# ns1labs/pktvisor

Hardware: AMD Instinct MI355X
Metric: Mpkt/s device-resident (Net+DNS handler parse) (higher is better)
Workload: dtype u8; 1 GPU; C2: Net+DNS handlers, 64 B UDP (Eth+IPv4+UDP+22 B), Zipf IPs, host_spec 10.x.x.x/8; records_per_gpu=10000000, handlers=net v1 + dns v1 (default groups), parallelism=dp1

## Files before the change

### include/pvgpu.h

```cpp
#ifndef PVGPU_H
#define PVGPU_H

#include <stddef.h>
#include <stdint.h>

#ifdef __cplusplus
extern "C" {
#endif

typedef struct pv_ctx pv_ctx;

enum pv_status {
    PV_OK = 0,
    PV_EINVAL = -1,
    PV_EHIP = -2,
    PV_ECAPACITY = -3,
    PV_EUNSUPPORTED = -4,
    PV_ENODEV = -5
};

enum pv_net_group { PV_NET_COUNTERS = 1u << 0, PV_NET_CARDINALITY = 1u << 1, PV_NET_TOP_GEO = 1u << 2, PV_NET_TOP_IPS = 1u << 3 };
enum pv_dns_group {
    PV_DNS_CARDINALITY = 1u << 0, PV_DNS_COUNTERS = 1u << 1, PV_DNS_QUANTILES = 1u << 2, PV_DNS_HISTOGRAMS = 1u << 3,
    PV_DNS_TRANSACTIONS = 1u << 4, PV_DNS_TOP_ECS = 1u << 5, PV_DNS_TOP_QNAMES = 1u << 6,
// ... 151 lines not shown
int pv_merge_hints(pv_ctx *ctx, uint64_t *open_queries, uint64_t *xact_values);
int pv_slow_values_export(pv_ctx *ctx, uint8_t **buf, size_t *bytes);
int pv_slow_finish(pv_ctx *ctx, const uint8_t *const *bufs, const size_t *sizes, uint32_t nranks);
int pv_values_export(pv_ctx *ctx, uint8_t **buf, size_t *bytes);
int pv_values_merge(pv_ctx *ctx, const uint8_t *buf, size_t bytes);
int pv_window_periods(pv_ctx *ctx, int part, uint32_t *slots, int64_t *start_sec, uint32_t max_n, uint32_t *n);
int pv_advance_windows(pv_ctx *ctx, int part, const int64_t *thresh, uint32_t n);
int pv_dns_event_seconds(pv_ctx *ctx, const uint8_t *d_recs, const uint32_t *d_offs, const pv_index_info *info,
                         const uint32_t *sc_idx, const uint32_t *sc_sec, int64_t *secs, uint32_t max, uint32_t *n);
int pv_plan_dns_draws(pv_ctx *ctx, uint64_t *draws);
int pv_sample_skip(pv_ctx *ctx, uint64_t net_draws, uint64_t dns_draws);
int pv_dns_event_seconds_host(pv_ctx *ctx, const uint8_t *recs, size_t bytes, int64_t *secs, uint32_t max, uint32_t *n);
int pv_shard_cuts(const uint8_t *recs, size_t bytes, const uint32_t *offs, uint64_t n, uint32_t linktype, uint32_t ts_nano,
                  uint32_t world, uint64_t *cuts);


int pv_set_start_tstamp(pv_ctx *ctx, int64_t sec, int64_t nsec);
int pv_set_end_tstamp(pv_ctx *ctx, int64_t sec, int64_t nsec);
int pv_synchronize(pv_ctx *ctx);
int pv_reset(pv_ctx *ctx);

int pv_window_json(pv_ctx *ctx, uint32_t period, int merged, char **out);
void pv_free(void *p);

#define PV_HANDLER_NET 1u
#define PV_HANDLER_DNS 2u
#define PV_PERIOD_AUTO 0xFFFFFFFFu
int pv_window_prometheus(pv_ctx *ctx, uint32_t period, uint32_t handlers, const char *const *label_keys,
                         const char *const *label_values, uint32_t n_labels, char **out);
int pv_window_opentelemetry(pv_ctx *ctx, uint32_t period, uint32_t handlers, const char *const *label_keys,
                            const char *const *label_values, uint32_t n_labels, uint8_t **out, size_t *bytes);
int pv_add_static_label(const char *key, const char *value);

int pv_check_period_shift(pv_ctx *ctx, int64_t sec, int64_t nsec);

typedef struct pv_bucket pv_bucket;
int pv_bucket_merge(pv_ctx *ctx, uint32_t handler, pv_bucket **bucket, uint32_t period, int prometheus, int merged);
int pv_bucket_json(pv_ctx *ctx, const pv_bucket *bucket, char **out);
int pv_bucket_prometheus(pv_ctx *ctx, const pv_bucket *bucket, const char *const *label_keys,
                         const char *const *label_values, uint32_t n_labels, char **out);
int pv_bucket_opentelemetry(pv_ctx *ctx, const pv_bucket *bucket, const char *const *label_keys,
                            const char *const *label_values, uint32_t n_labels, uint8_t **out, size_t *bytes);
void pv_bucket_free(pv_bucket *bucket);

int pv_state_regions(pv_ctx *ctx, void **sum_ptr, size_t *sum_bytes, void **min_ptr, size_t *min_bytes);
int pv_set_global_base(pv_ctx *ctx, uint64_t base);
enum pv_reduce_op { PV_REDUCE_SUM = 0, PV_REDUCE_MIN = 1 };
typedef struct pv_region {
    void *ptr;
    uint64_t words;
    uint32_t op;
    uint32_t pad;
} pv_region;
int pv_window_regions(pv_ctx *ctx, pv_region *regions, uint32_t max, uint32_t *n);

#define PV_COMM_ID_BYTES 128
int pv_comm_unique_id(uint8_t id[PV_COMM_ID_BYTES]);
int pv_comm_init(pv_ctx *ctx, const uint8_t id[PV_COMM_ID_BYTES], int nranks, int rank);
int pv_comm_allreduce_window(pv_ctx *ctx);
int pv_comm_allgather(pv_ctx *ctx, const void *buf, size_t bytes, uint8_t **out, uint64_t *sizes);
int pv_comm_destroy(pv_ctx *ctx);
int pv_export_topn(pv_ctx *ctx, uint8_t **buf, size_t *bytes);
int pv_merge_topn(pv_ctx *ctx, const uint8_t *buf, size_t bytes);

int pv_comm_merge_topn(pv_ctx *ctx);
int pv_topn_x_export(pv_ctx *ctx, uint32_t ranks, uint32_t rank, uint8_t **blob, size_t *bytes);
int pv_topn_x_import(pv_ctx *ctx, uint32_t ranks, uint32_t rank, const uint8_t *const *blobs, const size_t *sizes);
int pv_topn_x_candidates(pv_ctx *ctx, uint8_t **blob, size_t *bytes);
int pv_topn_x_names(pv_ctx *ctx, const uint8_t *const *cands, const size_t *sizes, uint32_t n, uint8_t **blob, size_t *bytes);
int pv_topn_x_view(pv_ctx *ctx, const uint8_t *const *cands, const size_t *csizes, const uint8_t *const *names,
                   const size_t *nsizes, uint32_t n);

typedef int (*pv_allreduce_fn)(uint64_t *buf, size_t n, int op, void *user);
int pv_values_x_select(pv_ctx *ctx, pv_allreduce_fn allreduce, void *user);
int pv_comm_values_select(pv_ctx *ctx);
int pv_slow_x_finish(pv_ctx *ctx, pv_allreduce_fn allreduce, void *user);
int pv_comm_slow_finish(pv_ctx *ctx);

int pv_set_kernel_timing(pv_ctx *ctx, uint32_t every);
const char *pv_net_kernel_name(pv_ctx *ctx);
int pv_kernel_timing(pv_ctx *ctx, double *total_ms, uint64_t *launches, int reset);
int pv_chain_stats(pv_ctx *ctx, uint64_t out[4], int reset);
int pv_fuse_stats(pv_ctx *ctx, uint64_t out[2], int reset);

typedef struct pv_geodb pv_geodb;
enum pv_geodb_kind { PV_GEODB_CITY = 0, PV_GEODB_ASN = 1 };
int pv_geodb_open(const uint8_t *bytes, size_t len, uint32_t kind, pv_geodb **db);
int pv_geodb_open_file(const char *path, uint32_t kind, pv_geodb **db);
void pv_geodb_close(pv_geodb *db);
const char *pv_geodb_last_error(void);
uint32_t pv_geodb_entries(const pv_geodb *db);
uint64_t pv_geodb_hash(const pv_geodb *db);
int pv_geodb_entry(const pv_geodb *db, uint32_t id, const char **name, const char **lat, const char **lon);
int pv_geodb_lookup(const pv_geodb *db, const uint8_t *addrs, size_t n, uint32_t addr_len, uint32_t *ids);
int pv_set_geodb(pv_ctx *ctx, const pv_geodb *city, const pv_geodb *asn);
typedef struct pv_net_filters {
    uint32_t geoloc_notfound;
    uint32_t asn_notfound;
    uint32_t only_geoloc_prefix_set;
    uint32_t n_geoloc_prefixes;
    const char *const *geoloc_prefixes;
    uint32_t only_asn_number_set;
    uint32_t n_asn_numbers;
    const char *const *asn_numbers;
} pv_net_filters;
int pv_set_net_filters(pv_ctx *ctx, const pv_net_filters *f);

#define PV_HANDLER_DHCP 4u
typedef struct pv_dhcp_config {
    uint32_t xact_ttl_ms;
    uint32_t recorded_stream;
    uint32_t max_events;
} pv_dhcp_config;
int pv_set_dhcp(pv_ctx *ctx, const pv_dhcp_config *cfg);
int pv_dhcp_timing(pv_ctx *ctx, double *scan_ms, uint64_t *launches, int reset);

#define PV_HANDLER_BGP 8u
typedef struct pv_bgp_config {
    uint32_t recorded_stream;
    uint32_t max_events;
} pv_bgp_config;
int pv_set_bgp(pv_ctx *ctx, const pv_bgp_config *cfg);
int pv_bgp_timing(pv_ctx *ctx, double *scan_ms, uint64_t *launches, int reset);
int pv_geodb_hashes(pv_ctx *ctx, uint64_t hashes[2]);
int pv_geodb_lookup_device(pv_ctx *ctx, uint32_t kind, const uint8_t *addrs, size_t n, uint32_t addr_len, uint32_t *ids);

#ifdef __cplusplus
}
#endif
#endif
```

### pktvisor_amd/__init__.py

```python
from __future__ import annotations

import ctypes
import json
import os
import struct
from typing import Optional

import numpy as np

HERE = os.path.dirname(os.path.abspath(__file__))
LIB_PATH = os.path.join(HERE, "libpvgpu.so")

PV_NET_COUNTERS, PV_NET_CARDINALITY, PV_NET_TOP_GEO, PV_NET_TOP_IPS = 1, 2, 4, 8
DNS_GROUPS = {"cardinality": 1 << 0, "counters": 1 << 1, "quantiles": 1 << 2, "histograms": 1 << 3,
              "dns_transaction": 1 << 4, "top_ecs": 1 << 5, "top_qnames": 1 << 6, "top_qnames_details": 1 << 7,
              "top_ports": 1 << 8}
NET_GROUPS = {"counters": 1, "cardinality": 2, "top_geo": 4, "top_ips": 8}
DNS_DEFAULT = sum(DNS_GROUPS[g] for g in ("cardinality", "counters", "quantiles", "dns_transaction", "top_qnames",
                                          "top_ports"))
NET_DEFAULT = 15


from pktvisor_amd.config import PvError

# ... 61 lines not shown
        if k in cfg and not isinstance(cfg[k], bool):
            raise ConfigError(f"wrong type for key: {k}")
    for k in ("only_qtype", "only_qname", "only_qname_suffix"):
        if k in cfg and (not isinstance(cfg[k], (list, tuple)) or not all(isinstance(x, str) for x in cfg[k])):
            raise ConfigError(f"wrong type for key: {k}")
    if cfg.get("exclude_noerror"):
        out["exclude_noerror"] = 1
    elif "only_rcode" in cfg:
        v = cfg["only_rcode"]
        if isinstance(v, bool) or not isinstance(v, (int, list, tuple)):
            raise ConfigError("DnsStreamHandler: wrong value type for only_rcode filter. It should be an integer or an array")
        if isinstance(v, int):
            if _dns_code(0, str(v)) is None:
                raise ConfigError("DnsStreamHandler: only_rcode filter contained an invalid/unsupported rcode")
            codes = [v]
        else:
            codes = []
            for r in v:
                c = _dns_code(0, r)
                if c is None:
                    raise ConfigError(f"DnsStreamHandler: only_rcode filter contained an invalid/unsupported rcode: {r}")
                codes.append(c)
        for c in codes:
            if c > 15:
                raise ConfigError("DnsStreamHandler: only_rcode filter contained an invalid/unsupported rcode")
            out["only_rcode_mask"] |= 1 << c
    if cfg.get("only_queries"):
        out["only_queries"] = 1
    if cfg.get("only_responses"):
        out["only_responses"] = 1
    if cfg.get("only_dnssec_response"):
        out["only_dnssec_response"] = 1
    if cfg.get("public_suffix_list"):
        out["public_suffix_list"] = 1
    if "answer_count" in cfg:
        v = cfg["answer_count"]
        if isinstance(v, bool) or not isinstance(v, int):
            raise ConfigError("DnsStreamHandler: wrong value type for answer_count filter. It should be an integer")
        out["answer_count"] = v
    for q in cfg.get("only_qtype", []):
        c = _dns_code(1, q)
        if c is None:
            raise ConfigError(f"DnsStreamHandler: only_qtype filter contained an invalid/unsupported qtype: {q}")
        out["only_qtype"].append(c)
    out["only_qname"] = [str(q).lower() for q in cfg.get("only_qname", [])]
    if out["only_qname"] and out["only_rcode_mask"] and not v2:
        raise ConfigError("DnsStreamHandler: only_qname and only_rcode both install an input predicate: use one")
    if len(out["only_qname"]) > 8 or any(not q or len(q) > 255 for q in out["only_qname"]):
        raise ConfigError("DnsStreamHandler: only_qname: 1..8 names of 1..255 characters")
    out["only_qname_suffix"] = [str(q).lower() for q in cfg.get("only_qname_suffix", [])]
    if len(out["only_qname_suffix"]) > 4:
        raise ConfigError("DnsStreamHandler: only_qname_suffix: at most 4 suffixes")
    if len(out["only_qtype"]) > 16:
        raise ConfigError("DnsStreamHandler: only_qtype: at most 16 qtypes")
    return out


class pv_index_info(ctypes.Structure):
    _fields_ = [("n_records", ctypes.c_uint64), ("bytes_used", ctypes.c_uint64), ("first_sec", ctypes.c_int64),
                ("first_nsec", ctypes.c_int64), ("last_sec", ctypes.c_int64), ("last_nsec", ctypes.c_int64),
                ("monotone", ctypes.c_uint32), ("n_sec_changes", ctypes.c_uint32)]


EXPORTS = ["pv_version", "pv_device_count", "pv_create", "pv_destroy", "pv_last_error", "pv_index_records",
           "pv_index_records_device",
           "pv_process_device", "pv_process_host", "pv_set_start_tstamp", "pv_set_end_tstamp", "pv_synchronize",
           "pv_reset", "pv_window_json", "pv_free", "pv_state_regions", "pv_set_global_base", "pv_export_topn",
           "pv_merge_topn", "pv_kernel_timing", "pv_set_kernel_timing", "pv_window_regions", "pv_index_records_mt", "pv_host_register",
           "pv_host_unregister", "pv_ingest_timing", "pv_edge_export", "pv_edge_merge", "pv_values_export",
           "pv_values_merge", "pv_window_periods", "pv_set_dns_filters", "pv_dns_code", "pv_advance_windows",
           "pv_dns_event_seconds", "pv_dns_event_seconds_host", "pv_comm_unique_id", "pv_comm_init",
           "pv_comm_allreduce_window", "pv_comm_allgather", "pv_comm_destroy", "pv_process_dnstap", "pv_dnstap_count",
           "pv_pcapng_records", "pv_tpacket3_block_records", "pv_window_prometheus", "pv_add_static_label",
           "pv_window_opentelemetry", "pv_check_period_shift", "pv_bucket_merge", "pv_bucket_json",
           "pv_bucket_prometheus", "pv_bucket_opentelemetry", "pv_bucket_free", "pv_set_slow_defer",
           "pv_slow_values_export", "pv_slow_finish", "pv_edge_carry", "pv_merge_hints", "pv_set_end_of_capture", "pv_shard_cuts", "pv_net_kernel_name",
           "pv_plan_dns_draws", "pv_sample_skip", "pv_set_tcp_reassembly_limit", "pv_set_tcp_exact_lru", "pv_set_dnstap_only_hosts",
           "pv_afpacket_open", "pv_afpacket_attach", "pv_afpacket_run", "pv_afpacket_start", "pv_afpacket_stop",
           "pv_afpacket_stats", "pv_afpacket_close", "pv_afpacket_last_error", "pv_set_bpf", "pv_bpf_validate",
           "pv_bpf_run", "pv_bpf_filter_records", "pv_comm_merge_topn", "pv_topn_x_export", "pv_topn_x_import",
           "pv_topn_x_candidates", "pv_topn_x_names", "pv_topn_x_view", "pv_values_x_select", "pv_comm_values_select",
           "pv_slow_x_finish", "pv_comm_slow_finish", "pv_geodb_open", "pv_geodb_open_file", "pv_geodb_close",
           "pv_geodb_last_error", "pv_geodb_entries", "pv_geodb_hash", "pv_geodb_hashes", "pv_set_net_filters", "pv_geodb_entry", "pv_geodb_lookup", "pv_set_geodb",
           "pv_geodb_lookup_device", "pv_set_dhcp", "pv_dhcp_timing", "pv_set_bgp", "pv_bgp_timing", "pv_chain_stats", "pv_fuse_stats"]
PV_GEODB_CITY, PV_GEODB_ASN = 0, 1
ALLREDUCE_FN = ctypes.CFUNCTYPE(ctypes.c_int, ctypes.POINTER(ctypes.c_uint64), ctypes.c_size_t, ctypes.c_int, ctypes.c_void_p)
PV_HANDLER_NET, PV_HANDLER_DNS, PV_HANDLER_DHCP, PV_HANDLER_BGP = 1, 2, 4, 8
_HANDLER_BITS = {"net": PV_HANDLER_NET, "dns": PV_HANDLER_DNS, "dhcp": PV_HANDLER_DHCP, "bgp": PV_HANDLER_BGP}
PV_PERIOD_AUTO = 0xFFFFFFFF
PART_NET, PART_DNS = 0, 1
PV_REDUCE_SUM, PV_REDUCE_MIN = 0, 1


class pv_bpf_insn(ctypes.Structure):
    _fields_ = [("code", ctypes.c_uint16), ("jt", ctypes.c_uint8), ("jf", ctypes.c_uint8), ("k", ctypes.c_uint32)]


def bpf_program(insns):
    arr = (pv_bpf_insn * max(1, len(insns)))()
    for i, (c, jt, jf, k) in enumerate(insns):
        arr[i] = pv_bpf_insn(c, jt, jf, k & 0xFFFFFFFF)
    return arr


def bpf_filter(recs: bytes, insns) -> bytes:
    lib = load_library()
    prog = bpf_program(insns)
    src = np.frombuffer(recs, dtype=np.uint8)
    out = np.empty(max(1, len(recs)), dtype=np.uint8)
    nb = ctypes.c_size_t()
    rc = lib.pv_bpf_filter_records(prog, len(insns), src.ctypes.data if len(recs) else None, len(recs), out.ctypes.data,
                                   ctypes.byref(nb), None)
    if rc:
        raise PvError(f"pv_bpf_filter_records failed ({rc}): invalid BPF program")
    return out[:nb.value].tobytes()


class pv_afpacket_config(ctypes.Structure):
    _fields_ = [("interface", ctypes.c_char_p), ("fanout_group_id", ctypes.c_int), ("block_size", ctypes.c_uint32),
                ("frame_size", ctypes.c_uint32), ("num_blocks", ctypes.c_uint32), ("bpf_insns", ctypes.c_void_p),
                ("bpf_len", ctypes.c_uint32), ("batch_bytes", ctypes.c_uint32), ("flush_ms", ctypes.c_uint32)]


class pv_afpacket_counters(ctypes.Structure):
    _fields_ = [(k, ctypes.c_uint64) for k in ("blocks", "packets", "batches", "bytes", "kernel_packets", "kernel_drops",
                                              "kernel_freezes")]


AFPACKET_SINK = ctypes.CFUNCTYPE(ctypes.c_int, ctypes.c_void_p, ctypes.c_void_p, ctypes.c_size_t, ctypes.c_uint64)


class pv_region(ctypes.Structure):
    _fields_ = [("ptr", ctypes.c_void_p), ("words", ctypes.c_uint64), ("op", ctypes.c_uint32), ("pad", ctypes.c_uint32)]

_lib = None


def load_library(path: str = LIB_PATH) -> ctypes.CDLL:
    global _lib
    if _lib is not None:
        return _lib
    path = os.environ.get("PVGPU_LIB", path)
    if not os.path.exists(path):
        raise PvError(f"{path} missing: run `make -C pktvisor_amd` (or __graft_entry__.build())")
    lib = ctypes.CDLL(path)
    P, U32, U64, I64 = ctypes.c_void_p, ctypes.c_uint32, ctypes.c_uint64, ctypes.c_int64
    lib.pv_version.restype = ctypes.c_char_p
    lib.pv_device_count.argtypes = [ctypes.POINTER(ctypes.c_int)]
    lib.pv_create.argtypes = [ctypes.POINTER(pv_config), ctypes.POINTER(P)]
    lib.pv_destroy.argtypes = [P]
    lib.pv_destroy.restype = None
    lib.pv_last_error.argtypes = [P]
    lib.pv_last_error.restype = ctypes.c_char_p
    lib.pv_index_records.argtypes = [P, ctypes.c_size_t, U32, P, U64, P, P, U32, ctypes.POINTER(pv_index_info)]
    lib.pv_index_records_device.argtypes = [P, P, ctypes.c_size_t, P, U64, P, P, U32, ctypes.POINTER(pv_index_info)]
    lib.pv_process_device.argtypes = [P, P, P, ctypes.POINTER(pv_index_info), P, P, P]
    lib.pv_index_records_mt.argtypes = [P, ctypes.c_size_t, U32, P, U64, P, P, U32, ctypes.POINTER(pv_index_info),
                                        U32]
    lib.pv_process_host.argtypes = [P, P, ctypes.c_size_t]
    lib.pv_host_register.argtypes = [P, ctypes.c_size_t]
    lib.pv_host_unregister.argtypes = [P]
    lib.pv_ingest_timing.argtypes = [P, ctypes.POINTER(ctypes.c_double), ctypes.c_int]
    lib.pv_set_start_tstamp.argtypes = [P, I64, I64]
    lib.pv_set_end_tstamp.argtypes = [P, I64, I64]
    lib.pv_synchronize.argtypes = [P]
    lib.pv_reset.argtypes = [P]
    lib.pv_window_json.argtypes = [P, U32, ctypes.c_int, ctypes.POINTER(P)]
# ... 24 lines not shown
    lib.pv_dns_event_seconds_host.argtypes = [P, P, ctypes.c_size_t, P, U32, ctypes.POINTER(U32)]
    lib.pv_kernel_timing.argtypes = [P, ctypes.POINTER(ctypes.c_double), ctypes.POINTER(U64), ctypes.c_int]
    lib.pv_set_kernel_timing.argtypes = [P, ctypes.c_uint32]
    lib.pv_edge_export.argtypes = [P, ctypes.POINTER(P), ctypes.POINTER(ctypes.c_size_t)]
    lib.pv_edge_merge.argtypes = [P, P, P, U32, U32]
    lib.pv_set_slow_defer.argtypes = [P, ctypes.c_int]
    lib.pv_plan_dns_draws.argtypes = [P, ctypes.POINTER(ctypes.c_uint64)]
    lib.pv_sample_skip.argtypes = [P, ctypes.c_uint64, ctypes.c_uint64]
    lib.pv_net_kernel_name.argtypes = [P]
    lib.pv_net_kernel_name.restype = ctypes.c_char_p
    lib.pv_shard_cuts.argtypes = [P, ctypes.c_size_t, P, ctypes.c_uint64, U32, U32, U32, P]
    lib.pv_edge_carry.argtypes = [P, P, ctypes.c_size_t, ctypes.POINTER(P), ctypes.POINTER(ctypes.c_size_t)]
    lib.pv_merge_hints.argtypes = [P, ctypes.POINTER(ctypes.c_uint64), ctypes.POINTER(ctypes.c_uint64)]
    lib.pv_set_end_of_capture.argtypes = [P, ctypes.c_int]
    lib.pv_slow_values_export.argtypes = [P, ctypes.POINTER(P), ctypes.POINTER(ctypes.c_size_t)]
    lib.pv_slow_finish.argtypes = [P, P, P, U32]
    lib.pv_values_export.argtypes = [P, ctypes.POINTER(P), ctypes.POINTER(ctypes.c_size_t)]
    lib.pv_values_merge.argtypes = [P, P, ctypes.c_size_t]
    lib.pv_window_periods.argtypes = [P, ctypes.c_int, P, P, U32, ctypes.POINTER(U32)]
    lib.pv_set_dns_filters.argtypes = [P, ctypes.POINTER(pv_dns_filters)]
    lib.pv_set_tcp_reassembly_limit.argtypes = [P, ctypes.c_uint64]
    lib.pv_set_tcp_exact_lru.argtypes = [P, ctypes.c_int]
    lib.pv_set_bpf.argtypes = [P, P, U32]
    lib.pv_bpf_validate.argtypes = [P, U32]
    lib.pv_bpf_run.argtypes = [P, P, U32, U32]
    lib.pv_bpf_run.restype = ctypes.c_uint32
    lib.pv_bpf_filter_records.argtypes = [P, U32, P, ctypes.c_size_t, P, ctypes.POINTER(ctypes.c_size_t), P]
    lib.pv_set_dnstap_only_hosts.argtypes = [P, ctypes.c_char_p]
    lib.pv_dns_code.argtypes = [ctypes.c_int, ctypes.c_char_p, ctypes.POINTER(U32)]
    lib.pv_comm_unique_id.argtypes = [P]
    lib.pv_comm_init.argtypes = [P, P, ctypes.c_int, ctypes.c_int]
    lib.pv_comm_allreduce_window.argtypes = [P]
    lib.pv_comm_allgather.argtypes = [P, P, ctypes.c_size_t, ctypes.POINTER(P), P]
    lib.pv_comm_destroy.argtypes = [P]
    lib.pv_comm_merge_topn.argtypes = [P]
    lib.pv_topn_x_export.argtypes = [P, U32, U32, ctypes.POINTER(P), ctypes.POINTER(ctypes.c_size_t)]
    lib.pv_topn_x_import.argtypes = [P, U32, U32, P, P]
    lib.pv_topn_x_candidates.argtypes = [P, ctypes.POINTER(P), ctypes.POINTER(ctypes.c_size_t)]
    lib.pv_topn_x_names.argtypes = [P, P, P, U32, ctypes.POINTER(P), ctypes.POINTER(ctypes.c_size_t)]
    lib.pv_topn_x_view.argtypes = [P, P, P, P, P, U32]
    lib.pv_values_x_select.argtypes = [P, ALLREDUCE_FN, P]
    lib.pv_comm_values_select.argtypes = [P]
    lib.pv_slow_x_finish.argtypes = [P, ALLREDUCE_FN, P]
    lib.pv_comm_slow_finish.argtypes = [P]
    lib.pv_process_dnstap.argtypes = [P, P, ctypes.c_size_t, U32]
    lib.pv_tpacket3_block_records.argtypes = [P, ctypes.c_size_t, P, ctypes.c_size_t, ctypes.POINTER(ctypes.c_size_t),
                                              ctypes.POINTER(U64)]
    lib.pv_pcapng_records.argtypes = [P, ctypes.c_size_t, P, ctypes.c_size_t, ctypes.POINTER(ctypes.c_size_t),
                                      ctypes.POINTER(U32), ctypes.POINTER(U64)]
    lib.pv_dnstap_count.argtypes = [P, ctypes.c_size_t, ctypes.POINTER(U32), ctypes.POINTER(U32)]
    lib.pv_afpacket_open.argtypes = [ctypes.POINTER(pv_afpacket_config), ctypes.POINTER(P)]
    lib.pv_afpacket_attach.argtypes = [P, U32, U32, ctypes.c_int, ctypes.POINTER(pv_afpacket_config), ctypes.POINTER(P)]
    lib.pv_afpacket_run.argtypes = [P, AFPACKET_SINK, P]
    lib.pv_afpacket_start.argtypes = [P, P]
    lib.pv_afpacket_stop.argtypes = [P]
    lib.pv_afpacket_stats.argtypes = [P, ctypes.POINTER(pv_afpacket_counters)]
    lib.pv_afpacket_close.argtypes = [P]
    lib.pv_afpacket_close.restype = None
    lib.pv_afpacket_last_error.restype = ctypes.c_char_p
    lib.pv_geodb_open.argtypes = [P, ctypes.c_size_t, U32, ctypes.POINTER(P)]
    lib.pv_geodb_open_file.argtypes = [ctypes.c_char_p, U32, ctypes.POINTER(P)]
    lib.pv_geodb_close.argtypes = [P]
    lib.pv_geodb_close.restype = None
    lib.pv_geodb_last_error.restype = ctypes.c_char_p
    lib.pv_geodb_entries.argtypes = [P]
    lib.pv_geodb_entries.restype = U32
    lib.pv_set_net_filters.argtypes = [P, ctypes.POINTER(pv_net_filters)]
    lib.pv_geodb_hashes.argtypes = [P, ctypes.POINTER(ctypes.c_uint64)]
    lib.pv_geodb_hash.argtypes = [P]
    lib.pv_geodb_hash.restype = U64
    lib.pv_geodb_entry.argtypes = [P, U32, ctypes.POINTER(ctypes.c_char_p), ctypes.POINTER(ctypes.c_char_p),
                                   ctypes.POINTER(ctypes.c_char_p)]
    lib.pv_geodb_lookup.argtypes = [P, P, ctypes.c_size_t, U32, P]
    lib.pv_set_geodb.argtypes = [P, P, P]
    lib.pv_geodb_lookup_device.argtypes = [P, U32, P, ctypes.c_size_t, U32, P]
    lib.pv_set_dhcp.argtypes = [P, ctypes.POINTER(pv_dhcp_config)]
    lib.pv_dhcp_timing.argtypes = [P, ctypes.POINTER(ctypes.c_double), ctypes.POINTER(U64), ctypes.c_int]
    lib.pv_set_bgp.argtypes = [P, ctypes.POINTER(pv_bgp_config)]
    lib.pv_bgp_timing.argtypes = [P, ctypes.POINTER(ctypes.c_double), ctypes.POINTER(U64), ctypes.c_int]
    if hasattr(lib, "pv_chain_stats"):
        lib.pv_chain_stats.argtypes = [P, ctypes.POINTER(U64), ctypes.c_int]
    if hasattr(lib, "pv_fuse_stats"):
        lib.pv_fuse_stats.argtypes = [P, ctypes.POINTER(U64), ctypes.c_int]
    _lib = lib
    return lib


def comm_unique_id() -> bytes:
    buf = ctypes.create_string_buffer(128)
    if load_library().pv_comm_unique_id(buf) != 0:
        raise PvError("pv_comm_unique_id failed")
    return buf.raw


def device_count() -> int:
    n = ctypes.c_int(0)
    load_library().pv_device_count(ctypes.byref(n))
    return n.value


def pcapng_records(data: bytes):
    lib = load_library()
    buf = np.frombuffer(data, dtype=np.uint8)
    nb, lt, nr = ctypes.c_size_t(0), ctypes.c_uint32(0), ctypes.c_uint64(0)
    rc = lib.pv_pcapng_records(buf.ctypes.data, buf.nbytes, None, 0, ctypes.byref(nb), ctypes.byref(lt), ctypes.byref(nr))
    if rc:
        raise PvError("Cannot open pcap/pcapng file" + (" (interfaces with different linktypes)" if rc == -7 else ""))
    out = np.empty(nb.value, dtype=np.uint8)
    rc = lib.pv_pcapng_records(buf.ctypes.data, buf.nbytes, out.ctypes.data, out.nbytes, ctypes.byref(nb),
                               ctypes.byref(lt), ctypes.byref(nr))
    if rc:
        raise PvError(f"pv_pcapng_records failed ({rc})")
    return lt.value, out.tobytes()


def read_pcap(path: str):
    with open(path, "rb") as f:
        data = f.read()
    if len(data) >= 12 and struct.unpack_from("<I", data, 0)[0] == 0x0A0D0D0A:
        lt, recs = pcapng_records(data)
        return lt, 1, recs
    if len(data) < 24:
        raise PvError("Cannot open pcap/pcapng file")
    magic = struct.unpack_from("<I", data, 0)[0]
    if magic not in (0xA1B2C3D4, 0xA1B23C4D):
        raise PvError("Cannot open pcap/pcapng file (only little-endian classic pcap is supported)")
    linktype = struct.unpack_from("<I", data, 20)[0]
    return linktype, int(magic == 0xA1B23C4D), data[24:]


def tpacket3_records(blocks, out_cap: int = 1 << 26) -> bytes:
    lib = load_library()
    out = np.empty(out_cap, dtype=np.uint8)
    used, n = ctypes.c_size_t(0), ctypes.c_uint64(0)
    for b in blocks:
        buf = np.frombuffer(b, dtype=np.uint8)
        rc = lib.pv_tpacket3_block_records(buf.ctypes.data, buf.nbytes, out.ctypes.data, out.nbytes, ctypes.byref(used),
                                           ctypes.byref(n))
        if rc:
            raise PvError(f"pv_tpacket3_block_records failed ({rc})")
    return out[: used.value].tobytes()


def dnstap_count(frames: bytes):
    nf, ne = ctypes.c_uint32(0), ctypes.c_uint32(0)
    buf = np.frombuffer(frames, dtype=np.uint8)
    load_library().pv_dnstap_count(buf.ctypes.data, buf.nbytes, ctypes.byref(nf), ctypes.byref(ne))
    return nf.value, ne.value


def dnstap_reader(path: str, periods: int = 1, only_hosts: Optional[list] = None, **kw) -> dict:
    with open(path, "rb") as f:
        frames = f.read()
    h = PvHandlers(num_periods=periods, **kw)
    try:
        if only_hosts is not None:
            h._check(h.lib.pv_set_dnstap_only_hosts(h.ctx, ",".join(only_hosts).encode()), "pv_set_dnstap_only_hosts")
        h.process_dnstap(frames)
        key = f"{1 if periods == 1 else periods}m"
        return {key: h.window_json(0 if periods == 1 else periods, merged=periods != 1)}
    finally:
        h.close()


def pcap_file_bytes(records: bytes, linktype: int = 1, ts_nano: int = 0) -> bytes:
    magic = 0xA1B23C4D if ts_nano else 0xA1B2C3D4
# ... 254 lines not shown
        self._host = host_spec.encode() if host_spec else None
        cfg = pv_config(self._host, num_periods, topn_count, xact_ttl_ms, net_groups, dns_groups, linktype, ts_nano,
                        device, table_log2, max_records, topn_percentile_threshold, net_filter_all, net2_groups,
                        dns2_groups, deep_sample_rate)
        self.num_periods = num_periods
        self.device = device
        self.ctx = ctypes.c_void_p()
        rc = self.lib.pv_create(ctypes.byref(cfg), ctypes.byref(self.ctx))
        if rc:
            msg = self.lib.pv_last_error(self.ctx).decode() if self.ctx else "pv_create"
            self.lib.pv_destroy(self.ctx)
            self.ctx = None
            raise PvError(f"pv_create failed ({rc}): {msg}")
        if filt:
            f = pv_dns_filters(filt["exclude_noerror"], filt["only_rcode_mask"], filt["answer_count"],
                               filt["only_queries"], filt["only_responses"], len(filt["only_qtype"]))
            for k, q in enumerate(filt["only_qtype"]):
                f.qtypes[k] = q
            f.only_dnssec_response = filt["only_dnssec_response"]
            f.filter_all = filt.get("filter_all", 0)
            f.public_suffix_list = filt.get("public_suffix_list", 0)
            f.v2 = filt.get("v2", 0)
            f.xact_dirs_disabled = filt.get("xact_dirs_disabled", 0)
            if filt["only_qname"]:
                self._qnames = (ctypes.c_char_p * len(filt["only_qname"]))(*[q.encode() for q in filt["only_qname"]])
                f.n_qnames = len(filt["only_qname"])
                f.qnames = ctypes.cast(self._qnames, ctypes.POINTER(ctypes.c_char_p))
            if filt["only_qname_suffix"]:
                sx = filt["only_qname_suffix"]
                self._qsfx = (ctypes.c_char_p * len(sx))(*[q.encode() for q in sx])
                f.n_qname_suffixes = len(sx)
                f.qname_suffixes = ctypes.cast(self._qsfx, ctypes.POINTER(ctypes.c_char_p))
            self._check(self.lib.pv_set_dns_filters(self.ctx, ctypes.byref(f)), "pv_set_dns_filters")
        self.tcp_exact = bool(tcp_exact_lru or tcp_packet_reassembly_cache_limit)
        if tcp_packet_reassembly_cache_limit:
            self._check(self.lib.pv_set_tcp_reassembly_limit(self.ctx, int(tcp_packet_reassembly_cache_limit)),
                        "pv_set_tcp_reassembly_limit")
        if tcp_exact_lru:
            self._check(self.lib.pv_set_tcp_exact_lru(self.ctx, 1), "pv_set_tcp_exact_lru")
        if bpf:
            self.set_bpf(bpf)
        if geo_city_db is not None or geo_asn_db is not None:
            self.set_geodb(geo_city_db, geo_asn_db)
        if net_filters:
            self.set_net_filters(**net_filters)
        self.dhcp_attached = False
        if dhcp is not None:
            self.set_dhcp(dhcp["xact_ttl_ms"], dhcp["recorded_stream"], dhcp_max_events)

        self.bgp_attached = False
        if bgp is not None:
            self.set_bgp(bgp["recorded_stream"], bgp_max_events)

    def set_bgp(self, recorded_stream: bool = False, max_events: int = 0):
        cfg = pv_bgp_config(int(bool(recorded_stream)), int(max_events))
        self._check(self.lib.pv_set_bgp(self.ctx, ctypes.byref(cfg)), "pv_set_bgp")
        self.bgp_attached = True

    def bgp_timing(self, reset: bool = False):
        ms, n = ctypes.c_double(), ctypes.c_uint64()
        self._check(self.lib.pv_bgp_timing(self.ctx, ctypes.byref(ms), ctypes.byref(n), int(reset)), "pv_bgp_timing")
        return ms.value, n.value

    def set_dhcp(self, xact_ttl_ms: int = 0, recorded_stream: bool = False, max_events: int = 0):
        cfg = pv_dhcp_config(int(xact_ttl_ms), int(bool(recorded_stream)), int(max_events))
        self._check(self.lib.pv_set_dhcp(self.ctx, ctypes.byref(cfg)), "pv_set_dhcp")
        self.dhcp_attached = True

    def dhcp_timing(self, reset: bool = False):
        ms, n = ctypes.c_double(), ctypes.c_uint64()
        self._check(self.lib.pv_dhcp_timing(self.ctx, ctypes.byref(ms), ctypes.byref(n), int(reset)), "pv_dhcp_timing")
        return ms.value, n.value

    def chain_stats(self, reset: bool = False):
        out = (ctypes.c_uint64 * 4)()
        self._check(self.lib.pv_chain_stats(self.ctx, out, int(reset)), "pv_chain_stats")
        return tuple(int(v) for v in out)

    def fuse_stats(self, reset: bool = False):
        out = (ctypes.c_uint64 * 2)()
        self._check(self.lib.pv_fuse_stats(self.ctx, out, int(reset)), "pv_fuse_stats")
        return tuple(int(v) for v in out)

    def set_net_filters(self, geoloc_notfound=False, asn_notfound=False, only_geoloc_prefix=None, only_asn_number=None):
        f = pv_net_filters(int(bool(geoloc_notfound)), int(bool(asn_notfound)))
        keep = []
        for name, lst in (("geoloc_prefixes", only_geoloc_prefix), ("asn_numbers", only_asn_number)):
            if lst is None:
                continue
            arr = (ctypes.c_char_p * max(1, len(lst)))(*[str(x).encode() for x in lst])
            keep.append(arr)
            setattr(f, name, ctypes.cast(arr, ctypes.POINTER(ctypes.c_char_p)))
            setattr(f, "n_" + name, len(lst))
            setattr(f, "only_geoloc_prefix_set" if name == "geoloc_prefixes" else "only_asn_number_set", 1)
        self._check(self.lib.pv_set_net_filters(self.ctx, ctypes.byref(f)), "pv_set_net_filters")

    def set_geodb(self, city=None, asn=None):
        own = []
        dbs = []
        for src, kind in ((city, "city"), (asn, "asn")):
            if src is not None and not isinstance(src, GeoDB):
                src = GeoDB(src, kind)
                own.append(src)
            dbs.append(src)
        try:
            self._check(self.lib.pv_set_geodb(self.ctx, dbs[0].ptr if dbs[0] else None, dbs[1].ptr if dbs[1] else None),
                        "pv_set_geodb")
            hs = (ctypes.c_uint64 * 2)()
            self._check(self.lib.pv_geodb_hashes(self.ctx, hs), "pv_geodb_hashes")
            self.geo_hashes = [int(hs[0]), int(hs[1])]
        finally:
            for d in own:
                d.close()

    def geo_lookup_device(self, kind: str, addrs, addr_len: int) -> np.ndarray:
        buf = _packed_addrs(addrs, addr_len)
        ids = np.empty(buf.size // addr_len, dtype=np.uint32)
        self._check(self.lib.pv_geodb_lookup_device(self.ctx, PV_GEODB_CITY if kind == "city" else PV_GEODB_ASN,
                                                    buf.ctypes.data, ids.size, addr_len, ids.ctypes.data),
                    "pv_geodb_lookup_device")
        return ids

    def set_bpf(self, insns):
        self._bpf = bpf_program(insns or [])
        self._check(self.lib.pv_set_bpf(self.ctx, self._bpf, len(insns or [])), "pv_set_bpf")

    def _check(self, rc, what):
        if rc:
            raise PvError(f"{what} failed ({rc}): {self.lib.pv_last_error(self.ctx).decode()}")

    def close(self):
        if self.ctx:
            self.lib.pv_destroy(self.ctx)
            self.ctx = None

    def __del__(self):
        try:
            self.close()
        except Exception:
            pass

    def process_host(self, recs):
        buf = recs if isinstance(recs, np.ndarray) else np.frombuffer(recs, dtype=np.uint8)
        self._check(self.lib.pv_process_host(self.ctx, buf.ctypes.data, buf.nbytes), "pv_process_host")

    def set_end_of_capture(self, on: bool = True):
        self._check(self.lib.pv_set_end_of_capture(self.ctx, int(on)), "pv_set_end_of_capture")

    def process_dnstap(self, frames):
        buf = frames if isinstance(frames, np.ndarray) else np.frombuffer(frames, dtype=np.uint8)
        self._check(self.lib.pv_process_dnstap(self.ctx, buf.ctypes.data, buf.nbytes, self.dnstap_mask),
                    "pv_process_dnstap")

    def index_device(self, recs, max_records: Optional[int] = None, max_changes: int = 1 << 16):
        buf = np.frombuffer(recs, dtype=np.uint8) if not isinstance(recs, np.ndarray) else recs
        if max_records is None:
            max_records = max(1, len(buf) // 16)
        offs = np.empty(max_records, dtype=np.uint32)
        sci = np.empty(max_changes, dtype=np.uint32)
        scs = np.empty(max_changes, dtype=np.uint32)
        info = pv_index_info()
        self._check(self.lib.pv_index_records_device(self.ctx, buf.ctypes.data, len(buf), offs.ctypes.data, max_records,
                                                     sci.ctypes.data, scs.ctypes.data, max_changes, ctypes.byref(info)),
                    "pv_index_records_device")
        return offs[: info.n_records], sci, scs, info

# ... 348 lines not shown
```

### pktvisor_amd/csrc/pv_host.cpp

```cpp
#include "pv_host.h"

namespace {

int parse_host_spec(pv_ctx *c, const char *spec)
{
    if (!spec) return 0;
    std::string s = spec;
    size_t pos = 0;
    while (pos < s.size()) {
        size_t e = s.find(',', pos);
        std::string host = s.substr(pos, e == std::string::npos ? std::string::npos : e - pos);
        pos = e == std::string::npos ? s.size() : e + 1;
        if (host.empty()) continue;
        size_t d = host.find('/');
        if (d == std::string::npos) return c->fail(PV_EINVAL, "invalid CIDR: %s", host.c_str());
        std::string ip = host.substr(0, d), cs = host.substr(d + 1);
        if (cs.empty() || !std::all_of(cs.begin(), cs.end(), ::isdigit)) return c->fail(PV_EINVAL, "invalid CIDR: %s", host.c_str());
        int cidr = atoi(cs.c_str());
        if (ip.find(':') != std::string::npos) {
            if (cidr < 0 || cidr > 128) return c->fail(PV_EINVAL, "invalid CIDR: %s", host.c_str());
            if (c->nets.n6 >= PV_MAX_SUBNETS) return c->fail(PV_EINVAL, "too many host subnets");
            uint8_t a[16];
            if (inet_pton(AF_INET6, ip.c_str(), a) != 1) return c->fail(PV_EINVAL, "invalid IPv6 address: %s", ip.c_str());
            memcpy(c->nets.v6_addr[c->nets.n6], a, 16);
// ... 2044 lines not shown
    P.iplog32 = c->d_iplog32;
    P.ipdir = c->d_ipdir;
    P.ipx_cnt = c->d_ipx_cnt;
    P.ipx_rep = c->d_ipx_rep;
    P.trash = c->d_trash;
    if ((uint64_t)grid * 4 > PV_TRASH_WAVES) return c->fail(PV_ECAPACITY, "grid of %u workgroups exceeds the trash area", grid);
    P.cb = c->d_cb;
    P.cb_cnt = c->d_cb_cnt;
    P.cb_hm = c->d_cb_cnt + 32768;
    P.stamps = c->d_stamps;
    P.dq = c->d_dq;
    P.dq_cnt = c->d_dq_cnt;
    static const char *force = getenv("PV_NET_KERNEL");
    const bool general = P.n_shift || P.net_filter_all || P.gfilt || P.dbg || P.ndeep_net || c->tcp_exact_on() ||
                         (force && !strcmp(force, "general"));
    const uint32_t reg_grid = std::min<uint32_t>(grid, (uint32_t)(c->cus * c->reg_wg_per_cu));
    const uint64_t per_wave = ((uint64_t)P.wt_per_block / 4 + 1) * ((grid + reg_grid - 1) / reg_grid);
    const bool lean = !general && P.linktype == 1 && P.nets.n4 <= 2 && P.skip_before == 0 && per_wave < 65535 &&
                      !(force && !strcmp(force, "ns"));
    P.ip_compact = lean ? 1u : 0u;
    P.ip_base = ((uint64_t)P.slot_of[0] << 60) | ((uint64_t)TM_IPV4 << 56) |
                ((uint64_t)((c->net_groups & PV_NET_CARDINALITY) ? 1 : 0) << 33);
    const bool tc = (c->dev_net_groups() & PV_NET_TOP_IPS) != 0;
    {
        const char *fan = getenv("PV_CB_FAN"), *cmp = getenv("PV_CB_COMPACT");
        P.cb_compact = cmp && atoi(cmp) == 0 ? 0u : 1u;
        uint32_t pick = c->cb_fan;
        if (P.cb_compact && lean && tc && !c->net2_groups && c->cb_plain) {
            const uint32_t f = std::min<uint32_t>(3u, 65535u / (P.wt_per_block * 64u));
            if (f > 1 && (grid + f - 1) / f >= (uint32_t)c->cus) pick = f;
        }
        P.cb_fan = fan ? std::max(1u, std::min(8u, (uint32_t)atoi(fan))) : pick;
        while (P.cb_fan > 1 && (uint64_t)P.cb_fan * P.mq_cap >= (1u << 24)) P.cb_fan--;
        P.cb_grid = (grid + P.cb_fan - 1) / P.cb_fan;
    }
    const bool span = lean && tc && force && !strcmp(force, "span");
    bool plain = lean && !(force && !strcmp(force, "span")) && c->cb_plain && !c->net2_groups && !c->geo_counting();
    if (plain) {
        const char *pc = getenv("PV_PLAIN_CHAIN");
        if (pc && atoi(pc) == 0) plain = false;
    }
    P.plain_chain = plain ? 1u : 0u;
    bool fuse = plain && tc && P.cb_fan > 1 && P.cb_grid == reg_grid && c->reg_log2 <= 10;
    if (fuse) {
        const char *fp = getenv("PV_FUSE_PLAIN");
        if (fp && atoi(fp) == 0) fuse = false;
    }
    {
        const char *nc = getenv("PV_NET_CONTIG");
        P.net_contig = nc && atoi(nc) != 0 && lean && P.cb_fan > 1 && P.cb_grid == reg_grid ? 1u : 0u;
    }
    if (lean) {
        if (c->slow_cap < P.n) {
            if (c->d_slow) hipFree(c->d_slow);
            c->d_slow = nullptr;
            c->slow_cap = 0;
            if (!hip_ok(e = hipMalloc(&c->d_slow, (size_t)(P.n + PV_MAX_GRID) * 4))) return c->hipfail(e, "deferred record list");
            c->slow_cap = P.n;
        }
        P.slow_list = c->d_slow;
        P.slow_cnt = c->d_slow + c->slow_cap;
    }
    if (c->dns_groups & PV_DNS_TOP_ECS) {
        if (c->ecs_cap < P.n) {
            if (c->d_ecs) hipFree(c->d_ecs);
            c->d_ecs = nullptr;
            c->ecs_cap = 0;
            if (!hip_ok(e = hipMalloc(&c->d_ecs, (size_t)P.n * sizeof(uint4)))) return c->hipfail(e, "top_ecs list");
            c->ecs_cap = P.n;
        }
        P.ecs_list = reinterpret_cast<uint32_t *>(c->d_ecs);
        P.ecs_cap = (uint32_t)c->ecs_cap;
    }
    *c->h_params = P;
    if (!hip_ok(e = fill_and_upload(c, c->d_params, c->h_params, sizeof P, st)))
        return c->hipfail(e, "parameter upload");
    c->net_kernel = general ? "pv_net_kernel"
                            : (lean ? (span ? "pv_net_kernel_span" : (tc ? "pv_net_kernel_reg_tc" : "pv_net_kernel_reg"))
                                    : "pv_net_kernel_ns");
    const PvParams *dp = (const PvParams *)c->d_params;
    const bool timed = n && c->timing_every && (c->timing_ctr++ % c->timing_every) == 0;
    hipEvent_t e0 = timed ? c->ev_start : nullptr, e1 = timed ? c->ev_stop : nullptr;
    if (timed) fuse = false;
    if (P.gfilt && n) {
        PvGeoArgs G{};
        for (int k = 0; k < 2; k++) {
            const pv_ctx::GeoAttach &g = c->geo[k];
            if (!g.on) continue;
            G.tree[k] = g.d_tree;
            G.node_count[k] = g.node_count;
            G.start4[k] = g.start4;
            G.ip_version[k] = g.ip_version;
            G.entries[k] = (uint32_t)g.dict.size();
        }
        hipLaunchKernelGGL(pv_geo_verdict, dim3((uint32_t)((P.n + 255) / 256)), dim3(256), 0, st, dp, G,
                           (const uint8_t *)(c->nf_on[0] ? c->d_nf_pass[0] : nullptr),
                           (const uint8_t *)(c->nf_on[1] ? c->d_nf_pass[1] : nullptr), c->d_gfilt);
    }
    if (!n) {  }
    else if (general) hipExtLaunchKernelGGL(pv_net_kernel, dim3(grid), dim3(PV_NET_THREADS), 0, st, e0, e1, 0, dp);
    else if (lean) {
        hipEvent_t l1 = plain ? e1 : (hipEvent_t) nullptr;
        if (fuse) hipLaunchKernelGGL(pv_net_combine_plain, dim3(P.cb_grid), dim3(PV_CB_THREADS), 0, st, dp);
        else if (span) hipExtLaunchKernelGGL(pv_net_kernel_span, dim3(reg_grid), dim3(PV_NET_THREADS), 0, st, e0, l1, 0, dp);
        else if (tc) hipExtLaunchKernelGGL(pv_net_kernel_reg_tc, dim3(reg_grid), dim3(PV_NET_THREADS), 0, st, e0, l1, 0, dp);
        else hipExtLaunchKernelGGL(pv_net_kernel_reg, dim3(reg_grid), dim3(PV_NET_THREADS), 0, st, e0, l1, 0, dp);
        if (!plain) hipExtLaunchKernelGGL(pv_net_slow_list, dim3(c->cus * 2), dim3(256), 0, st, (hipEvent_t) nullptr, e1, 0, dp);
    }
    else hipExtLaunchKernelGGL(pv_net_kernel_ns, dim3(grid), dim3(PV_NET_THREADS), 0, st, e0, e1, 0, dp);
    e = hipGetLastError();
    if (e != hipSuccess) return c->hipfail(e, "launch pv_net_kernel");
    static int cb_threads = 0;
    if (!cb_threads) {
        hipFuncAttributes fa{};
        cb_threads = hipFuncGetAttributes(&fa, reinterpret_cast<const void *>(pv_topn_combine)) == hipSuccess ? fa.maxThreadsPerBlock
                                                                                                             : PV_CB_THREADS;
    }
    const bool sfx = (P.f_flags & (PVDF_ONLY_QSUFFIX | PVDF_PSL)) != 0;
    auto dns_stage = [&]() {
        if (sfx) hipLaunchKernelGGL(pv_dns_suffix, dim3(grid), dim3(256), 0, st, (const PvParams *)c->d_params);
        const uint32_t dns_grid = std::min<uint32_t>(grid, (uint32_t)(c->cus * c->dns_wg_per_cu));
        if (sfx)
            hipLaunchKernelGGL(pv_dns_kernel_sfx, dim3(dns_grid), dim3(64 * PV_DNS_WAVES), 0, st, (const PvParams *)c->d_params);
        else if (P.f_flags)
            hipLaunchKernelGGL(pv_dns_kernel_f, dim3(dns_grid), dim3(64 * PV_DNS_WAVES), 0, st, (const PvParams *)c->d_params);
        else
            hipLaunchKernelGGL(pv_dns_kernel, dim3(dns_grid), dim3(64 * PV_DNS_WAVES), 0, st, (const PvParams *)c->d_params);
        if (c->dns_groups & PV_DNS_TOP_ECS)
            hipLaunchKernelGGL(pv_dns_ecs, dim3((uint32_t)c->cus * 2), dim3(256), 0, st, (const PvParams *)c->d_params);
        if (c->net2_groups) hipLaunchKernelGGL(pv_net2_kernel, dim3(grid), dim3(256), 0, st, (const PvParams *)c->d_params);
    };
    auto topn_stage = [&](bool combined = false) {
        if (!combined)
            hipLaunchKernelGGL(c->reg_log2 <= 10 ? pv_topn_combine : pv_topn_combine_r12, dim3(P.cb_grid), dim3(cb_threads), 0, st,
                               (const PvParams *)c->d_params);
        if (c->geo_counting()) {
            PvGeoArgs G{};
            for (int k = 0; k < 2; k++) {
                const pv_ctx::GeoAttach &g = c->geo[k];
                if (!g.on) continue;
                G.tree[k] = g.d_tree;
                G.cnt[k] = g.d_cnt;
                G.node_count[k] = g.node_count;
                G.start4[k] = g.start4;
                G.ip_version[k] = g.ip_version;
                G.entries[k] = (uint32_t)g.dict.size();
            }
            hipLaunchKernelGGL(pv_geo_count, dim3(std::min<uint32_t>(P.cb_grid, (uint32_t)c->cus * 8)), dim3(256), 0, st,
                               (const PvParams *)c->d_params, G);
        }
        hipLaunchKernelGGL(pv_topn_merge, dim3(2u << c->reg_log2), dim3(pv_topn_merge_threads()), 0, st, (const PvParams *)c->d_params);
    };
    auto names_stage = [&]() {
        hipLaunchKernelGGL(sfx ? pv_topn_names_sfx : pv_topn_names, dim3((uint32_t)c->cus * 2), dim3(256), 0, st,
                           (const PvParams *)c->d_params);
    };
    uint32_t status[ST_WORDS];
    auto read_status = [&]() -> hipError_t {
        hipError_t r = hipGetLastError();
        if (r != hipSuccess) return r;
        if ((r = hipMemcpyAsync(c->h_status, c->d_status, ST_RB_WORDS * 4, hipMemcpyDeviceToHost, st)) != hipSuccess) return r;
        if ((r = hipStreamSynchronize(st)) != hipSuccess) return r;
        memcpy(status, c->h_status, sizeof status);
        return hipSuccess;
    };
    if (!n) {
    } else if (!plain) {
        dns_stage();
        topn_stage();
        names_stage();
        c->chain_n[3]++;
    } else {
        topn_stage(fuse);
        c->chain_n[0]++;
        if (fuse) c->fuse_n[0]++;
    }

    HP(14);
    if (!hip_ok(e = read_status())) return c->hipfail(e, "kernel execution");
    if (plain && (status[ST_NDNS] || status[ST_NSLOW])) {
        c->chain_n[1]++;
        if (fuse) c->fuse_n[1]++;
        P.plain_chain = 0;
        c->h_params->plain_chain = 0;
        if (!hip_ok(e = upload_params(c->d_params, c->h_params, sizeof P, st))) return c->hipfail(e, "parameter upload");
        hipLaunchKernelGGL(pv_net_slow_list, dim3(c->cus * 2), dim3(256), 0, st, dp);
        dns_stage();
        topn_stage();
        names_stage();
        if (!hip_ok(e = read_status())) return c->hipfail(e, "kernel execution");
    } else if (plain && status[ST_NNEW]) {
        c->chain_n[2]++;
        names_stage();
        if (!hip_ok(e = read_status())) return c->hipfail(e, "kernel execution");
    }
    if (n) {
        c->dns_heavy = (uint64_t)status[ST_NDNS] * 2 > n;
        c->cb_plain = lean && status[ST_NDNS] == 0 && status[ST_NSLOW] == 0;
    }
    if (status[ST_FLAGS] & PVF_NAMES_PENDING) {
        for (uint32_t t = 0; t < PV_TABLES; t++)
            hipLaunchKernelGGL(pv_topn_name_fix, dim3((uint32_t)c->cus * 4), dim3(256), 0, st, (const PvParams *)c->d_params, t);
        if (!hip_ok(e = hipGetLastError()) || !hip_ok(e = hipStreamSynchronize(st))) return c->hipfail(e, "pending names");
        if (getenv("PV_NAMEFIX_TRACE")) fprintf(stderr, "pv: pending top-N names written (pv_topn_name_fix)\n");
    }
    HP(4);
    {
        float ms = 0;
        if (timed && hipEventElapsedTime(&ms, c->ev_start, c->ev_stop) == hipSuccess) { c->kernel_ms += ms; c->kernel_launches++; }
    }
    if (!c->tcp_pre) {
        if (int rc = tcp_stage(c, d_recs, d_offs, n, status[ST_TSEG], status[ST_TSEG_BYTES], first_sec, false, st)) return rc;
    }
    const uint32_t gt = tcp_pass(c, P, a, a + nord, st, c->h_params + 1);
    if (gt) {
        if (P.want_events)
            hipLaunchKernelGGL(pv_xact_compact, dim3(gt), dim3(256), 0, st, (const PvParams *)c->d_params, grid,
                               status[ST_NKEYS]);
        if (!hip_ok(e = hipGetLastError())) return c->hipfail(e, "launch pv_dns_tcp");
        if (!hip_ok(e = hipMemcpyAsync(c->h_status, c->d_status, ST_RB_WORDS * 4, hipMemcpyDeviceToHost, st)) ||
            !hip_ok(e = hipStreamSynchronize(st)))
            return c->hipfail(e, "TCP DNS pass");
        memcpy(status, c->h_status, sizeof status);
    }
    for (uint32_t k = 0; k <= P.n_shift; k++) c->net.clean[P.slot_of[k]] = false;
    if (status[ST_NDNS] || gt)
        for (uint32_t k = 0; k <= P.n_dshift; k++) c->dns.clean[P.dslot_of[k]] = false;
    bool drained = false;
    if (int rc = drain_overflow(c, st, true, &drained)) return rc;
    uint32_t flags = status[ST_FLAGS];
    if (drained && !hip_ok(e = hipMemcpy(&flags, c->d_status + ST_FLAGS, 4, hipMemcpyDeviceToHost))) return c->hipfail(e, "status");
    if (flags & PVF_TABLE_FULL) return c->fail(PV_ECAPACITY, "top-N table full: raise table_log2");
    if (flags & PVF_ARENA_FULL) return c->fail(PV_ECAPACITY, "top-N name arena full");
    if (getenv("PV_TSTAMPS")) {
        std::vector<uint64_t> tv(65536 + (2u << c->reg_log2) * 8);
        if (hip_ok(hipMemcpy(tv.data(), c->d_stamps + (1u << 20), tv.size() * 8, hipMemcpyDeviceToHost))) {
            double cs[8] = {0}, ms[8] = {0};
            uint64_t nm = 0;
            const uint32_t cg = P.cb_grid;
            for (uint32_t w = 0; w < cg; w++)
                for (int k = 0; k < 8; k++) cs[k] += (double)tv[w * 8 + k];
            for (uint32_t w = 0; w < (2u << c->reg_log2); w++) {
                const uint64_t *m = &tv[65536 + w * 8];
                if (!m[0] && !m[1]) continue;
                nm++;
                for (int k = 0; k < 8; k++) ms[k] += (double)m[k];
            }
            fprintf(stderr, "pv_tstamps combine (%u wg): init=%.0f insert=%.0f count=%.0f scan=%.0f out=%.0f | merge (%lu wg): "
                            "runs=%.0f load=%.0f insert=%.0f names=%.0f wb=%.0f\n",
                    cg, cs[0] / cg, cs[1] / cg, cs[2] / cg, cs[3] / cg, cs[4] / cg, (unsigned long)nm,
                    ms[0] / std::max<uint64_t>(nm, 1), ms[1] / std::max<uint64_t>(nm, 1), ms[2] / std::max<uint64_t>(nm, 1),
                    ms[3] / std::max<uint64_t>(nm, 1), ms[4] / std::max<uint64_t>(nm, 1));
            hipMemset(c->d_stamps + (1u << 20), 0, tv.size() * 8);
        }
        std::vector<uint64_t> nv((size_t)reg_grid * 4);
        int khz = 0;
        hipDeviceGetAttribute(&khz, hipDeviceAttributeWallClockRate, c->device);
        if (lean && hip_ok(hipMemcpy(nv.data(), c->d_stamps + (1u << 20) + (1u << 18), nv.size() * 8, hipMemcpyDeviceToHost)) && nv[0]) {
            uint64_t first = ~0ull;
            for (uint32_t w = 0; w < reg_grid; w++) first = std::min(first, nv[w * 4]);
            const double us = khz > 0 ? 1000.0 / khz : 0.01;
            fprintf(stderr, "pv_tstamps net (%u wg, %s):", reg_grid, fuse ? "fused" : "pair");
            static const char *nm[4] = {"start", "net_end", "handover", "end"};
            for (int k = 0; k < (fuse ? 4 : 2); k++) {
                std::vector<double> v;
                for (uint32_t w = 0; w < reg_grid; w++)
                    if (nv[w * 4 + k]) v.push_back((double)(nv[w * 4 + k] - first) * us);
                if (v.empty()) continue;
                std::sort(v.begin(), v.end());
                fprintf(stderr, " %s min=%.2f med=%.2f max=%.2f us", nm[k], v.front(), v[v.size() / 2], v.back());
            }
            fprintf(stderr, "\n");
            hipMemset(c->d_stamps + (1u << 20) + (1u << 18), 0, nv.size() * 8);
        }
    }
    if (getenv("PV_STAMPS")) {
        std::vector<uint64_t> stv((size_t)grid * 4 * 8);
        if (hip_ok(hipMemcpy(stv.data(), c->d_stamps, stv.size() * 8, hipMemcpyDeviceToHost))) {
            double sum[8] = {0};
            for (size_t w = 0; w < (size_t)grid * 4; w++)
                for (int k = 0; k < 8; k++) sum[k] += (double)stv[w * 8 + k];
            fprintf(stderr, "pv_stamps (mean cycles per wave, %u wave tiles/wg):", P.wt_per_block);
            static const char *nm[8] = {"slot", "commit", "barA", "issue", "parse", "lane", "barB", "flush"};
            for (int k = 0; k < 8; k++) fprintf(stderr, " %s=%.0f", nm[k], sum[k] / (grid * 4.0));
            fprintf(stderr, "\n");
        }
    }
    HP(5);
    if (int rc = pair_stage(c, P, status[ST_NEV], status[ST_NKEYS], status[ST_NRESP], n, st,
                            (uint64_t)(grid + gt) * P.wt_per_block * 64u))
        return rc;
    HP(6);
    const bool ovf_known = c->ovf_known;
    c->ovf_known = false;
    if ((status[ST_NEV] || c->n_pend) && P.want_events)
        if (int rc = drain_overflow(c, st, ovf_known)) return rc;

    for (const Shift &sh : nsh) win_shift(c, c->net, sh.sec);
    for (const Shift &sh : dsh) {
        win_shift(c, c->dns, sh.sec);
        c->dns_shifts.emplace_back(sh.sec, c->dns.slot_at(0));
        c->dns_shift_ord.emplace_back(sh.sec, c->dns.ordinal);
    }
    c->records_seen += n;
    const int prc = purge_tables(c, st);
    HP(7);
    return prc;
}

int batch_shifts(pv_ctx *c, const uint8_t *d_recs, const uint32_t *d_offs, const pv_index_info *info,
                 const uint32_t *sc_idx, const uint32_t *sc_sec, hipStream_t st, std::vector<Shift> &nsh,
                 std::vector<Shift> &dsh)
{
    c->tcp_pre = false;
    c->tcp_nmsg = 0;
    c->tcp_ords.clear();
    c->tcp_items.clear();
    int64_t top = info->last_sec;
    if (!info->monotone)
        for (uint32_t k = 0; k < info->n_sec_changes; k++) top = std::max<int64_t>(top, (int64_t)sc_sec[k]);
    if (c->sample_rate < 100) {
        c->tcp_pre = true;
        uint32_t tseg[2] = {0, 0};
        if (int rc = dns_prescan(c, d_recs, d_offs, info->n_records, st, true, tseg)) return rc;
        const bool dns_may = c->cfg.num_periods > 1 && top >= c->dns.next_shift_sec;
        c->eoc_stage = c->eoc_batch;
        if (int rc = tcp_stage(c, d_recs, d_offs, info->n_records, tseg[0], tseg[1], (uint32_t)info->first_sec, true, st))
            return rc;
        if (c->cfg.num_periods <= 1) return 0;
        const bool net_may = top >= c->net.next_shift_sec;
        if (!net_may && !dns_may) return 0;
        if (net_may) net_shifts_of(c->net.next_shift_sec, info, sc_idx, sc_sec, nsh);
        if (dns_may) dns_shifts_of(c->dns.next_shift_sec, c->h_dbits, info->n_records, info, sc_idx, sc_sec, c->tcp_ords, dsh);
        return 0;
    }
    if (c->cfg.num_periods <= 1) return 0;
    const bool net_may = top >= c->net.next_shift_sec, dns_may = top >= c->dns.next_shift_sec;
    if (!net_may && !dns_may) return 0;
    if (net_may) net_shifts_of(c->net.next_shift_sec, info, sc_idx, sc_sec, nsh);
    c->tcp_pre = dns_may || nsh.size() > PV_MAX_SHIFTS;
    if (c->tcp_pre) {
        uint32_t tseg[2] = {0, 0};
        if (int rc = dns_prescan(c, d_recs, d_offs, info->n_records, st, true, tseg)) return rc;
        c->eoc_stage = c->eoc_batch;
        if (int rc = tcp_stage(c, d_recs, d_offs, info->n_records, tseg[0], tseg[1], (uint32_t)info->first_sec, dns_may, st))
            return rc;
    }
    if (dns_may) dns_shifts_of(c->dns.next_shift_sec, c->h_dbits, info->n_records, info, sc_idx, sc_sec, c->tcp_ords, dsh);
    return 0;
}

int flush_empty(pv_ctx *c, hipStream_t st)
{
// ... 150 lines not shown
    }
    const uint32_t total = tail[0] + tail[1];
    for (uint32_t base = 0; base < total; base += c->dhcp_cap) {
        const uint32_t k = std::min(c->dhcp_cap, total - base);
        uint32_t top = 0;
        if (!hip_ok(e = hipMemsetAsync(c->d_dh_top, 0, 4, st))) return c->hipfail(e, "DHCP decode");
        hipLaunchKernelGGL(pv_dhcp_decode, dim3((n + 255) / 256), dim3(256), 0, st, d_recs, d_offs, n, c->cfg.linktype,
                           c->cfg.ts_nano, (const PvParams *)c->d_dh_params, (const unsigned long long *)c->d_dh_mask,
                           (const uint32_t *)c->d_dh_rank, base, c->dhcp_cap, c->d_dh_ev, c->d_dh_arena,
                           c->dhcp_cap * PV_DHCP_HOST_MAX, c->d_dh_top);
        if (!hip_ok(e = hipGetLastError())) return c->hipfail(e, "launch pv_dhcp_decode");
        c->h_dh_ev.resize(k);
        if (!hip_ok(e = hipMemcpyAsync(c->h_dh_ev.data(), c->d_dh_ev, (size_t)k * sizeof(PvDhcpEvent), hipMemcpyDeviceToHost, st)) ||
            !hip_ok(e = hipMemcpyAsync(&top, c->d_dh_top, 4, hipMemcpyDeviceToHost, st)) || !hip_ok(e = hipStreamSynchronize(st)))
            return c->hipfail(e, "DHCP events");
        top = std::min(top, c->dhcp_cap * PV_DHCP_HOST_MAX);
        c->h_dh_arena.resize(top);
        if (top && !hip_ok(e = hipMemcpy(c->h_dh_arena.data(), c->d_dh_arena, top, hipMemcpyDeviceToHost)))
            return c->hipfail(e, "DHCP hostnames");
        c->dhcp->replay(c->h_dh_ev.data(), k, c->h_dh_arena.data(), top);
    }
    return 0;
}

static void dhcp_free(pv_ctx *c)
{
    for (void *p : {(void *)c->d_dh_mask, (void *)c->d_dh_cnt, (void *)c->d_dh_rank, (void *)c->d_dh_top, (void *)c->d_dh_ev,
                    (void *)c->d_dh_arena, (void *)c->d_dh_params, c->d_dh_scan})
        if (p) hipFree(p);
    c->d_dh_mask = nullptr;
    c->d_dh_cnt = c->d_dh_rank = c->d_dh_top = nullptr;
    c->d_dh_ev = nullptr;
    c->d_dh_arena = nullptr;
    c->d_dh_params = nullptr;
    c->d_dh_scan = nullptr;
    c->dh_scan_bytes = 0;
    c->dhcp.reset();
}

extern "C" int pv_set_dhcp(pv_ctx *c, const pv_dhcp_config *cfg)
{
    std::lock_guard<std::mutex> g(c->mu);
    if (c->started) return c->fail(PV_EINVAL, "pv_set_dhcp: call before the first batch");
    hipSetDevice(c->device);
    dhcp_free(c);
    if (!cfg) return 0;
    c->dhcp_cfg = *cfg;
    const uint64_t maxn = std::max<uint64_t>(1, c->max_records);
    uint64_t cap = cfg->max_events ? cfg->max_events : std::min<uint64_t>(maxn, 1u << 20);
    cap = std::min<uint64_t>(cap, 1u << 22);
    c->dhcp_cap = (uint32_t)cap;
    const size_t ntiles = (size_t)((maxn + 63) / 64);
    hipError_t e;
    size_t tb = 0;
    if (!hip_ok(e = hipMalloc(&c->d_dh_mask, ntiles * 8)) || !hip_ok(e = hipMalloc(&c->d_dh_cnt, ntiles * 4)) ||
        !hip_ok(e = hipMalloc(&c->d_dh_rank, ntiles * 4)) || !hip_ok(e = hipMalloc(&c->d_dh_top, 256)) ||
        !hip_ok(e = hipMalloc(&c->d_dh_ev, cap * sizeof(PvDhcpEvent))) ||
        !hip_ok(e = hipMalloc(&c->d_dh_arena, cap * PV_DHCP_HOST_MAX)) || !hip_ok(e = hipMalloc(&c->d_dh_params, sizeof(PvParams))) ||
        !hip_ok(e = hipMemset(c->d_dh_params, 0, sizeof(PvParams))) ||
        !hip_ok(e = pv_exclusive_scan_u32(nullptr, &tb, nullptr, nullptr, ntiles, c->stream))) {
        dhcp_free(c);
        return c->hipfail(e, "DHCP stage buffers");
    }
    if (int rc = x_grow_dev(c, &c->d_dh_scan, c->dh_scan_bytes, tb, "DHCP scan")) { dhcp_free(c); return rc; }
    c->dhcp.reset(new pvdhcp::Manager(c->cfg.num_periods, c->cfg.deep_sample_rate, cfg->xact_ttl_ms));
    return 0;
}

extern "C" int pv_dhcp_timing(pv_ctx *c, double *scan_ms, uint64_t *launches, int reset)
{
    std::lock_guard<std::mutex> g(c->mu);
    if (scan_ms) *scan_ms = c->dhcp_scan_ms;
    if (launches) *launches = c->dhcp_scan_launches;
    if (reset) { c->dhcp_scan_ms = 0; c->dhcp_scan_launches = 0; }
    return 0;
}

extern "C" int pv_fuse_stats(pv_ctx *c, uint64_t out[2], int reset)
{
    std::lock_guard<std::mutex> g(c->mu);
    for (int k = 0; k < 2; k++) {
        if (out) out[k] = c->fuse_n[k];
        if (reset) c->fuse_n[k] = 0;
    }
    return 0;
}

extern "C" int pv_chain_stats(pv_ctx *c, uint64_t out[4], int reset)
{
    std::lock_guard<std::mutex> g(c->mu);
    for (int k = 0; k < 4; k++) {
        if (out) out[k] = c->chain_n[k];
        if (reset) c->chain_n[k] = 0;
    }
    return 0;
}

static int bgp_stage(pv_ctx *c, const uint8_t *d_recs, const uint32_t *d_offs, const pv_index_info *info, hipStream_t st)
{
    hipError_t e;
    const uint32_t n = (uint32_t)info->n_records, ntiles = (n + 63) / 64;
    size_t tb = 0, tb2 = 0;
    if (!hip_ok(e = pv_exclusive_scan_u32(nullptr, &tb, nullptr, nullptr, ntiles, st)) ||
        !hip_ok(e = pv_bgp_prefix_max(nullptr, &tb2, nullptr, nullptr, ntiles, st)))
        return c->hipfail(e, "BGP scan size");
    if (int rc = x_grow_dev(c, &c->d_bg_scan, c->bg_scan_bytes, std::max(tb, tb2), "BGP scan")) return rc;
    const uint32_t grid = std::max(1u, std::min((ntiles + 3) / 4, (uint32_t)c->cus * 8));
    const bool timed = c->timing_every != 0;
    if (timed) hipEventRecord(c->ev_start, st);
    hipLaunchKernelGGL(pv_bgp_scan, dim3(grid), dim3(256), 0, st, d_recs, d_offs, n, c->cfg.linktype, c->cfg.ts_nano,
                       (const PvParams *)c->d_bg_params, c->d_bg_mask, c->d_bg_cnt, c->d_bg_tsec);
    if (!hip_ok(e = hipGetLastError())) return c->hipfail(e, "launch pv_bgp_scan");
    if (timed) hipEventRecord(c->ev_stop, st);
    tb = c->bg_scan_bytes;
    uint32_t tail[3] = {0, 0, 0};
    if (!hip_ok(e = pv_exclusive_scan_u32(c->d_bg_scan, &tb, c->d_bg_cnt, c->d_bg_rank, ntiles, st))) return c->hipfail(e, "BGP scan");
    tb = c->bg_scan_bytes;
    if (!hip_ok(e = pv_bgp_prefix_max(c->d_bg_scan, &tb, c->d_bg_tsec, c->d_bg_tincl, ntiles, st)) ||
        !hip_ok(e = hipMemcpyAsync(&tail[0], c->d_bg_rank + ntiles - 1, 4, hipMemcpyDeviceToHost, st)) ||
        !hip_ok(e = hipMemcpyAsync(&tail[1], c->d_bg_cnt + ntiles - 1, 4, hipMemcpyDeviceToHost, st)) ||
        !hip_ok(e = hipMemcpyAsync(&tail[2], c->d_bg_tincl + ntiles - 1, 4, hipMemcpyDeviceToHost, st)) ||
        !hip_ok(e = hipStreamSynchronize(st)))
        return c->hipfail(e, "BGP scan");
    if (timed) {
        float ms = 0;
        if (hipEventElapsedTime(&ms, c->ev_start, c->ev_stop) == hipSuccess) { c->bgp_scan_ms += ms; c->bgp_scan_launches++; }
    }
    const uint32_t total = tail[0] + tail[1];
    uint32_t kmax = c->bgp_cap;
    for (uint32_t base = 0; base < total;) {
        uint32_t k = std::min(kmax, total - base);
        unsigned long long top = 0;
        for (;;) {
            if (!hip_ok(e = hipMemsetAsync(c->d_bg_top, 0, 8, st))) return c->hipfail(e, "BGP decode");
            hipLaunchKernelGGL(pv_bgp_decode, dim3((n + 255) / 256), dim3(256), 0, st, d_recs, d_offs, n, c->cfg.linktype,
                               c->cfg.ts_nano, (const PvParams *)c->d_bg_params, (const unsigned long long *)c->d_bg_mask,
                               (const uint32_t *)c->d_bg_rank, (const uint32_t *)c->d_bg_tincl, base, k, c->d_bg_seg, c->d_bg_arena,
                               c->bgp_arena_cap, c->d_bg_top);
            if (!hip_ok(e = hipGetLastError())) return c->hipfail(e, "launch pv_bgp_decode");
            if (!hip_ok(e = hipMemcpyAsync(&top, c->d_bg_top, 8, hipMemcpyDeviceToHost, st)) || !hip_ok(e = hipStreamSynchronize(st)))
                return c->hipfail(e, "BGP decode");
            if (top <= c->bgp_arena_cap || k == 1) break;
            k = (k + 1) / 2;
            kmax = k;
        }
        if (top > c->bgp_arena_cap) return c->fail(PV_EINVAL, "BGP decode: a segment of %llu bytes", top);
        c->h_bg_seg.resize(k);
        c->h_bg_arena.resize((size_t)top);
        if (!hip_ok(e = hipMemcpyAsync(c->h_bg_seg.data(), c->d_bg_seg, (size_t)k * sizeof(PvBgpSeg), hipMemcpyDeviceToHost, st)) ||
            (top && !hip_ok(e = hipMemcpyAsync(c->h_bg_arena.data(), c->d_bg_arena, (size_t)top, hipMemcpyDeviceToHost, st))) ||
            !hip_ok(e = hipStreamSynchronize(st)))
            return c->hipfail(e, "BGP segments");
        c->bgp->replay(c->h_bg_seg.data(), k, c->h_bg_arena.data(), (size_t)top);
        base += k;
    }
    c->bgp->end_batch(tail[2]);
    if (c->eoc_batch) c->bgp->close_all();
    return 0;
}

static void bgp_free(pv_ctx *c)
{
    for (void *p : {(void *)c->d_bg_mask, (void *)c->d_bg_top, (void *)c->d_bg_cnt, (void *)c->d_bg_rank, (void *)c->d_bg_tsec,
                    (void *)c->d_bg_tincl, (void *)c->d_bg_seg, (void *)c->d_bg_arena, (void *)c->d_bg_params, c->d_bg_scan})
        if (p) hipFree(p);
    c->d_bg_mask = c->d_bg_top = nullptr;
// ... 1369 lines not shown
```

### pktvisor_amd/csrc/pv_host.h

```cpp
#pragma once
#include <hip/hip_runtime.h>
#include <hip/hip_ext.h>
#include <rccl/rccl.h>

#include <algorithm>
#include <array>
#include <arpa/inet.h>
#include <linux/if_packet.h>
#include <cmath>
#include <cstdarg>
#include <cstdio>
#include <cstdlib>
#include <cctype>
#include <cstring>
#include <deque>
#include <list>
#include <map>
#include <mutex>
#include <sstream>
#include <string>
#include <unordered_map>
#include <queue>
#include <set>
#include <tuple>
// ... 34 lines not shown
        uint32_t h = 0x811C9DC5u;
        for (const char *x = k; *x; x++) h = (h ^ (uint8_t)*x) * 16777619u;
        uint32_t s = h & (PV_PSL_SLOTS - 1);
        while (w[s * 4 + 2]) s = (s + 1) & (PV_PSL_SLOTS - 1);
        w[s * 4] = h; w[s * 4 + 2] = (uint32_t)strlen(k); w[s * 4 + 1] = put(k);
        w[s * 4 + 3] = first | ((uint32_t)pv_psl_count[t] << 16);
        first += pv_psl_count[t];
    }
    for (uint32_t j = 0; j < PV_PSL_NSFX; j++) {
        w[PV_PSL_SFX_WORD + 2 * j + 1] = (uint32_t)strlen(pv_psl_sfx[j]);
        w[PV_PSL_SFX_WORD + 2 * j] = put(pv_psl_sfx[j]);
    }
    str.resize((str.size() + 3) & ~(size_t)3, '\0');
    const size_t n0 = w.size();
    w.resize(n0 + str.size() / 4);
    memcpy(w.data() + n0, str.data(), str.size());
    return w;
}
inline uint64_t name_ph(const char *s, size_t n)
{
    uint64_t ph = 0;
    for (size_t k = 0; k < n; k++) ph = ph_step(ph, lower((uint8_t)s[k]));
    return ph;
}
struct HostRecs {
    const uint8_t *p;
    size_t n;
    uint32_t u8(uint64_t o) const { return o < n ? p[o] : 0u; }
    uint32_t u32(uint64_t o) const
    {
        uint32_t v = 0;
        for (int k = 0; k < 4; k++) v |= u8(o + k) << (8 * k);
        return v;
    }
};
inline bool tcp_dns_flow(const HostRecs &R, const PvParams &P, uint64_t rec, uint32_t *key)
{
    Parsed o;
    parse_record(R, parse_cfg(P), P, rec, o);
    if (o.l4 != 6) return false;
    const uint32_t pw = R.u32(o.l4off);
    auto bs = [](uint32_t x) { return ((x & 0xff) << 8) | ((x >> 8) & 0xff); };
    const uint32_t sp = bs(pw & 0xffff), dp = bs(pw >> 16);
    auto dns = [](uint32_t x) { return x == 53 || x == 5353 || x == 5355 || x == 53000; };
    if (!dns(sp) && !dns(dp)) return false;
    *key = flowkey(R, o);
    return true;
}
inline uint64_t name_fp(const char *s, size_t n)
{
    NameStats st;
    st.init();
    for (size_t k = 0; k < n; k++) st.put((uint8_t)s[k]);
    return fp56(st.ph, st.n, 0);
}
#undef PV_FN
#undef PV_CREF
}

extern "C" __global__ void pv_net_kernel(const PvParams *P);
extern "C" __global__ void pv_net_kernel_ns(const PvParams *P);
extern "C" __global__ void pv_net_kernel_reg(const PvParams *P);
extern "C" __global__ void pv_net_kernel_reg_tc(const PvParams *P);
extern "C" __global__ void pv_net_kernel_span(const PvParams *P);
extern "C" __global__ void pv_store_blob(PvBlob b, uint4 *dst, uint32_t n16);
extern "C" __global__ void pv_fill_store(PvFillList L, PvBlob b, uint4 *dst, uint32_t n16);
extern "C" __global__ void pv_net_slow_list(const PvParams *P);
extern "C" __global__ void pv_rec_sizes(const uint8_t *recs, const uint32_t *offs, const uint8_t *trecs, const uint32_t *toffs,
                                        const uint32_t *idx, uint32_t stride, uint32_t n, uint32_t *sizes);
extern "C" __global__ void pv_rec_gather(const uint8_t *recs, const uint32_t *offs, const uint8_t *trecs, const uint32_t *toffs,
                                         const uint32_t *idx, uint32_t stride, uint32_t n, const uint32_t *dst_off, uint8_t *out);
extern "C" __global__ void pv_dns_kernel(const PvParams *P);
extern "C" __global__ void pv_dns_kernel_sfx(const PvParams *P);
extern "C" __global__ void pv_dns_kernel_f(const PvParams *P);
extern "C" __global__ void pv_dns_ecs(const PvParams *P);
extern "C" __global__ void pv_dns_suffix(const PvParams *P);
extern "C" __global__ void pv_fill_u64(uint64_t *p, uint64_t n, uint64_t v);
extern "C" __global__ void pv_fill_u32(uint32_t *p, uint64_t n, uint32_t v);
extern "C" __global__ void pv_fill_multi(PvFillList L);
extern "C" __global__ void pv_xact_compact(const PvParams *P, uint32_t b0, uint32_t kbase);
extern "C" __global__ void pv_dns_prescan(const PvParams *P);
extern "C" __global__ void pv_topn_combine(const PvParams *P);
extern "C" __global__ void pv_net_combine_plain(const PvParams *P);
extern "C" __global__ void pv_topn_combine_r12(const PvParams *P);
extern "C" __global__ void pv_topn_merge(const PvParams *P);
extern "C" __global__ void pv_topn_names_sfx(const PvParams *P);
extern "C" __global__ void pv_topn_name_fix(const PvParams *P, uint32_t tb);
extern "C" uint32_t pv_topn_merge_threads();
extern "C" __global__ void pv_geo_walk(const uint32_t *tree, uint32_t node_count, uint32_t start, const uint32_t *addrs, uint64_t n,
                                       uint32_t addr_words, uint32_t *ids);
extern "C" __global__ void pv_geo_count(const PvParams *P, PvGeoArgs G);
extern "C" __global__ void pv_geo_verdict(const PvParams *P, PvGeoArgs G, const uint8_t *pass_city, const uint8_t *pass_asn,
                                          unsigned long long *out);
struct PvBpfIns;
extern "C" __global__ void pv_bpf_keep(const uint8_t *recs, const uint32_t *offs, uint32_t n, const PvBpfIns *prog, uint32_t ninsn,
                                       uint32_t *sz, uint32_t *kf);
extern "C" __global__ void pv_bpf_gather(const uint8_t *recs, const uint32_t *offs, uint32_t n, const uint32_t *sz, const uint32_t *boff,
                                         const uint32_t *rank, uint8_t *out, uint32_t *ooffs);
extern "C" __global__ void pv_bpf_secs(const uint8_t *out, const uint32_t *ooffs, uint32_t nk, uint32_t *flag, uint32_t *sec, uint32_t *down);
extern "C" __global__ void pv_bpf_secs_compact(const uint32_t *flag, const uint32_t *pos, const uint32_t *sec, uint32_t nk, uint32_t cap,
                                               uint32_t *sci, uint32_t *scs);
extern "C" hipError_t pv_exclusive_scan_u32(void *tmp, size_t *tmp_bytes, const uint32_t *in, uint32_t *out, size_t n, hipStream_t s);
extern "C" __global__ void pv_dhcp_scan(const uint8_t *recs, const uint32_t *offs, uint32_t n, uint32_t linktype, uint32_t ts_nano,
                                        const PvParams *P, unsigned long long *mask, uint32_t *cnt);
extern "C" __global__ void pv_dhcp_decode(const uint8_t *recs, const uint32_t *offs, uint32_t n, uint32_t linktype, uint32_t ts_nano,
                                          const PvParams *P, const unsigned long long *mask, const uint32_t *rank, uint32_t base,
                                          uint32_t cap, PvDhcpEvent *ev, uint8_t *arena, uint32_t arena_cap, uint32_t *arena_top);
extern "C" __global__ void pv_bgp_scan(const uint8_t *recs, const uint32_t *offs, uint32_t n, uint32_t linktype, uint32_t ts_nano,
                                       const PvParams *P, unsigned long long *mask, uint32_t *cnt, uint32_t *tsec);
extern "C" hipError_t pv_bgp_prefix_max(void *tmp, size_t *tmp_bytes, const uint32_t *in, uint32_t *out, size_t n, hipStream_t s);
extern "C" __global__ void pv_bgp_decode(const uint8_t *recs, const uint32_t *offs, uint32_t n, uint32_t linktype, uint32_t ts_nano,
                                         const PvParams *P, const unsigned long long *mask, const uint32_t *rank, const uint32_t *tincl,
                                         uint32_t base, uint32_t cap, PvBgpSeg *seg, uint8_t *arena, uint32_t arena_cap,
                                         unsigned long long *arena_top);
extern "C" __global__ void pv_topn_xcount(const PvParams *P, PvXTabs T, uint32_t *cnt);
extern "C" __global__ void pv_topn_xscan(uint32_t reg_log2, uint32_t W, const uint32_t *cnt, uint32_t *off, uint32_t *hdr);
extern "C" __global__ void pv_topn_xwrite(const PvParams *P, PvXTabs T, const uint32_t *off, ulonglong2 *out);
extern "C" __global__ void pv_topn_xruns(uint32_t reg_log2, uint32_t W, uint32_t me, const uint32_t *hdr, uint32_t hdr_stride,
                                         uint64_t *cb_run);
extern "C" __global__ void pv_topn_xlookup(const PvParams *P, const uint64_t *keys, const uint32_t *tbs, uint32_t n, uint32_t *aux);
extern "C" __global__ void pv_net2_kernel(const PvParams *P);
extern "C" __global__ void pv_ix_guess(const PvIxParams *X);
extern "C" __global__ void pv_xv_hist(const PvXValue *v, const uint32_t *n_vals, uint32_t cap, uint32_t sg, uint32_t shift, PvXvSel sel,
                                      uint32_t *hist);
extern "C" __global__ void pv_ix_fix(const PvIxParams *X, uint32_t src);
extern "C" __global__ void pv_ix_scan(const PvIxParams *X);
extern "C" __global__ void pv_ix_write(const PvIxParams *X);
extern "C" __global__ void pv_ix_secs(const PvIxParams *X, uint32_t cap);
extern "C" __global__ void pv_ix_cut(const PvIxParams *X);
extern "C" __global__ void pv_topn_retry(const PvParams *P, const PvOvf *src, uint32_t n);
extern "C" __global__ void pv_xname_len(const uint8_t *arena, uint64_t arena_cap, const uint32_t *tb, const uint32_t *aux, uint32_t n,
                                        uint32_t *len);
extern "C" __global__ void pv_xname_copy(const uint8_t *arena, uint64_t arena_cap, const uint32_t *tb, const uint32_t *aux,
                                         const uint32_t *len, const uint64_t *off, uint32_t n, uint8_t *out);
extern "C" __global__ void pv_dns_tcp_filter(const PvParams *P);
extern "C" __global__ void pv_topn_purge(const PvParams *P, uint32_t tb, uint32_t *theta_out);
extern "C" __global__ void pv_topn_compact(const PvParams *P, uint32_t tb, uint8_t *tmp, unsigned long long *tmp_top);
extern "C" __global__ void pv_topn_names(const PvParams *P);
extern "C" __global__ void pv_xact_resolve(const PvXactParams *X);
extern "C" __global__ void pv_xact_resolve2(const PvXactParams *X);
extern "C" __global__ void pv_xact_slow_dev(const PvXactParams *X);
extern "C" __global__ void pv_xact_slow(const PvXactParams *X, uint32_t n_valid);
extern "C" __global__ void pv_xact_carry(const PvXactParams *X);
extern "C" __global__ void pv_xact_edge2(const PvXactParams *X, const PvEdgePair *pairs, uint32_t n, uint8_t *sfx, uint8_t *tsfx);
extern "C" __global__ void pv_xact_defer(const uint64_t *skeys, const uint32_t *svals, const PvXEvent *events, uint32_t n,
                                         PvXEvent *pend, uint64_t *pkeys, uint32_t *pvals, uint32_t at, uint32_t ehi,
                                         const uint64_t *eecs, uint64_t *pecs, uint32_t *ctr);
extern "C" __global__ void pv_xact_pend_in(uint64_t *skeys, uint32_t *svals, const uint64_t *pkeys, const uint32_t *pvals,
                                           uint32_t n_pend, uint32_t at);
extern "C" hipError_t pv_radix_sort_pairs(void *tmp, size_t *tmp_bytes, uint64_t *kin, uint64_t *kout, uint32_t *vin,
                                          uint32_t *vout, size_t n, hipStream_t s);
extern "C" __global__ void pv_dns_tcp(const PvParams *P);
extern "C" __global__ void pv_dnstap_kernel(const PvParams *P);
extern "C" __global__ void pv_tcp_keys(const PvTcpSeg *seg, uint32_t n, uint64_t *key, uint32_t *val);
extern "C" __global__ void pv_tcp_scan(const PvTcpParams *T);
extern "C" __global__ void pv_tcp_lookup(const PvTcpParams *T);
extern "C" __global__ void pv_tcp_insert(const PvTcpParams *T);
extern "C" __global__ void pv_tcp_flow(const PvTcpParams *T);
extern "C" __global__ void pv_tcp_migrate(const PvTcpParams *T);
extern "C" __global__ void pv_tcp_eoc(const PvTcpParams *T, const PvTcpSeg *seg, uint32_t n_seg, uint64_t *set, uint32_t set_mask,
                                      PvTcpSeg *out, uint32_t *cnt, uint32_t idx, uint32_t sec, uint32_t usec, uint32_t dir);
extern "C" __global__ void pv_tcp_keep_last(const uint8_t *recs, const uint32_t *offs, uint32_t n, uint8_t *out);
extern "C" hipError_t pv_tcp_sort(void *tmp, size_t *tmp_bytes, uint64_t *kin, uint64_t *kout, uint32_t *vin, uint32_t *vout,
                                  size_t n, hipStream_t s);

namespace pvh {
// ... 316 lines not shown
    bool nf_on[2] = {false, false};
    std::vector<std::string> nf_prefix[2];
    uint8_t *d_nf_pass[2] = {nullptr, nullptr};
    bool nf_ready = false;
    unsigned long long *d_gfilt = nullptr;
    bool nf_all() const { return (nf_on[0] && !geo[0].on) || (nf_on[1] && !geo[1].on); }
    bool nf_verdicts() const { return (nf_on[0] || nf_on[1]) && !nf_all() && !cfg.net_filter_all; }
    bool geo_counting() const { return (geo[0].on || geo[1].on) && (net_groups & PV_NET_TOP_GEO); }
    uint32_t dev_net_groups() const { return net_groups | (geo_counting() ? (uint32_t)PV_NET_TOP_IPS : 0u); }
    std::unique_ptr<pvdhcp::Manager> dhcp;
    pv_dhcp_config dhcp_cfg{};
    uint32_t dhcp_cap = 0;
    unsigned long long *d_dh_mask = nullptr;
    uint32_t *d_dh_cnt = nullptr, *d_dh_rank = nullptr, *d_dh_top = nullptr;
    PvDhcpEvent *d_dh_ev = nullptr;
    uint8_t *d_dh_arena = nullptr;
    PvParams *d_dh_params = nullptr;
    void *d_dh_scan = nullptr;
    size_t dh_scan_bytes = 0;
    std::vector<PvDhcpEvent> h_dh_ev;
    std::vector<uint8_t> h_dh_arena;
    double dhcp_scan_ms = 0;
    uint64_t dhcp_scan_launches = 0;
    std::vector<pv_bpf_insn> bpf;
    pv_bpf_insn *d_bpf = nullptr;
    size_t d_bpf_n = 0;
    bool bpf_dirty = false;
    uint32_t *d_fwork = nullptr;
    uint8_t *d_frecs = nullptr;
    uint32_t *d_foffs = nullptr, *d_fsc = nullptr;
    void *d_fscan = nullptr;
    size_t fwork_n = 0, frecs_bytes = 0, fscan_bytes = 0;
    pv_config cfg{};
    std::string err;
    std::mutex mu;
    int device = 0;
    hipStream_t stream = nullptr;
    PvSubnets nets{};
    uint32_t ttl_s = 0, ttl_ms = 0;
    uint32_t net_groups = PV_NET_DEFAULT_GROUPS, dns_groups = PV_DNS_DEFAULT_GROUPS;
    uint32_t net2_groups = 0;
    uint32_t dns2_groups = 0;
    float p90_2[3] = {0.0f, 0.0f, 0.0f};
    uint64_t *d_sum = nullptr;
    int64_t *d_cpc = nullptr;
    uint64_t *d_tkeys = nullptr, *d_tcnt = nullptr;
    uint32_t *d_taux = nullptr;
    uint8_t *d_arena = nullptr;
    uint64_t *d_arena_top = nullptr;
    uint64_t arena_cap = 128ull << 20;
    uint32_t tcap_log2 = 22;
    PvXEvent *d_events = nullptr;
    uint64_t *d_ekeys = nullptr;
    uint32_t *d_blk_events = nullptr;
    uint64_t *d_mq = nullptr;
    uint64_t *d_tpbuf = nullptr;
    uint64_t *d_cb = nullptr;
    uint32_t *d_cb_cnt = nullptr;
    uint32_t *d_cb_h = nullptr;
    uint32_t cb_h_grid = 0;
    PvNewName *d_nn = nullptr;
    uint64_t *d_iplog = nullptr;
    uint32_t *d_iplog32 = nullptr, *d_ipx_cnt = nullptr, *d_ipx_rep = nullptr;
    uint64_t *d_ipdir = nullptr;
    uint32_t *d_slow = nullptr;
    uint64_t slow_cap = 0;
    uint4 *d_ecs = nullptr;
    uint64_t ecs_cap = 0;
    uint64_t *d_trash = nullptr;
    uint32_t nn_cap = 0;
    uint32_t reg_log2 = 0;
    size_t mq_bytes = 0;
    uint32_t *d_mq_cnt = nullptr;
    uint64_t *d_stamps = nullptr;
    int cus = 256;
    int wg_per_cu = 3;
    bool wg_forced = false;
    bool dns_heavy = false;
    int reg_wg_per_cu = 1;
    uint32_t cb_fan = 1;
    bool cb_plain = false;
    uint64_t chain_n[4] = {0, 0, 0, 0};
    uint64_t fuse_n[2] = {0, 0};
    int dns_wg_per_cu = 1;
    const char *net_kernel = "none";
    uint64_t *d_dq = nullptr;
    uint32_t *d_dq_cnt = nullptr;
    uint64_t *d_skeys = nullptr, *d_skeys2 = nullptr;
    uint32_t *d_svals = nullptr, *d_svals2 = nullptr;
    void *d_sort_tmp = nullptr;
    size_t sort_tmp_bytes = 0;
    PvXValue *d_xvals = nullptr;
    uint64_t xv_cap = 0;
    uint32_t *d_xvh = nullptr, *h_xvh = nullptr;
    PvXValid *d_valid = nullptr;
    uint32_t *d_nvals = nullptr;
    PvXEvent *d_pend[2] = {nullptr, nullptr};
    uint64_t *d_eecs = nullptr, *d_pecs[2] = {nullptr, nullptr};
    uint64_t *d_pkeys[2] = {nullptr, nullptr};
    uint32_t *d_pvals[2] = {nullptr, nullptr};
    uint32_t pend_cur = 0;
    uint64_t n_pend = 0, pend_cap = 0;
    uint64_t ev_store_cap = 0, pend_hi = 0, key_cap = 0;
    int64_t pend_base = -1;
    PvXEvent *d_orph = nullptr;
    uint32_t orph_cap = 0;
    std::vector<std::pair<int64_t, uint32_t>> dns_shifts;
    uint32_t gen[PV_SLOTS] = {0};
    uint64_t *d_dbits = nullptr;
    uint64_t *h_dbits = nullptr;
    size_t xvals_synced = 0;
    float from90 = 0.0f, to90 = 0.0f;
    uint32_t *d_status = nullptr;
    uint32_t *d_tab_live = nullptr, *h_tab_live = nullptr, *d_theta = nullptr;
    PvOvf *d_ovf = nullptr, *d_ovf2 = nullptr;
    uint32_t *d_ovf_cnt = nullptr, ovf_cap = 0;
    uint32_t *h_ovf = nullptr;
    bool ovf_known = false;
    uint64_t ovf_rounds = 0;
    uint8_t *d_ctmp = nullptr;
    unsigned long long *d_ctop = nullptr;
    std::vector<uint64_t> roff[PV_TABLES];
    uint64_t purges = 0;
    uint32_t f_flags = 0, f_rcode_mask = 0, f_ancount = 0, f_nq = 0;
    uint16_t f_qt[PV_MAX_QTYPES] = {};
    uint32_t f_nqn = 0;
    uint64_t f_qn[PV_MAX_QNAMES] = {};
    uint8_t *d_sfx = nullptr;
    uint32_t *d_psl = nullptr;
    uint32_t f_nsx = 0, f_sxl[PV_MAX_SUFFIXES] = {};
    uint64_t f_sxh[PV_MAX_SUFFIXES] = {};
    PvParams *d_params = nullptr;
    PvParams *h_params = nullptr;
    PvXactParams *h_xparams = nullptr;
    uint32_t *h_status = nullptr;
    PvXactParams *d_xparams = nullptr;
    uint64_t max_records = 0;
    struct Stage {
        uint8_t *h_recs = nullptr, *d_recs = nullptr;
        uint32_t *h_offs = nullptr, *d_offs = nullptr;
        hipEvent_t copied = nullptr;
        std::vector<uint32_t> sci, scs;
        pv_index_info info{};
        uint8_t *d_ix = nullptr;
        PvIxParams *h_ix = nullptr;
        uint32_t ix_nseg = 0;
        uint32_t cut_o[2] = {0, 0};
        bool last = false;
    };
    bool device_index = true;
    struct Ring {
        uint8_t *d_buf = nullptr;
        uint32_t *d_offs = nullptr;
        uint8_t *h_stage = nullptr;
        hipEvent_t landed = nullptr;
    } ring[8];
    uint32_t ring_n = 4;
    hipStream_t copy_stream2 = nullptr;
    std::unique_ptr<pvi::Pool> pool;
    Stage stage[2];
    size_t stage_bytes = 0;
    uint64_t stage_recs = 0;
    hipStream_t copy_stream = nullptr;
    double ingest_ms[4] = {0, 0, 0, 0};
    bool hprof_on = getenv("PV_HOST_PROF") != nullptr;
    double hprof[20] = {};
// ... 178 lines not shown
```

### pktvisor_amd/csrc/pv_kernels.hip

```cpp
#include <cstring>
#include <hip/hip_runtime.h>
#include <rocprim/rocprim.hpp>
#include <stdint.h>

#include "pv_layout.h"
#include "pv_geodb.h"

#define PV_BLOCK 256
#define PV_C __attribute__((address_space(4)))
#ifdef PV_STAMPS
#define STAMP_DECL                                                                           \
    uint64_t st_acc[8] = {0, 0, 0, 0, 0, 0, 0, 0};                                          \
    uint64_t st_prev = __builtin_amdgcn_s_memtime();
#define STAMP(k)                                                                             \
    {                                                                                        \
        const uint64_t now = __builtin_amdgcn_s_memtime();                                   \
        st_acc[k] += now - st_prev;                                                          \
        st_prev = now;                                                                       \
    }
#define STAMP_FLUSH                                                                          \
    if ((threadIdx.x & 63) == 0)                                                             \
        for (int k_ = 0; k_ < 8; k_++) P.stamps[((uint64_t)blockIdx.x * (blockDim.x / 64) + threadIdx.x / 64) * 8 + k_] = st_acc[k_];
#else
#define STAMP_DECL
#define STAMP(k)
#define STAMP_FLUSH
#endif
#ifdef PV_TSTAMPS
#define TST_DECL uint64_t tst_prev = __builtin_amdgcn_s_memtime(), tst_acc[8] = {0, 0, 0, 0, 0, 0, 0, 0};
#define TST(k)                                                                               \
    {                                                                                        \
        const uint64_t now = __builtin_amdgcn_s_memtime();                                   \
        tst_acc[k] += now - tst_prev;                                                        \
        tst_prev = now;                                                                      \
    }
#define TST_FLUSH(base)                                                                      \
    if (threadIdx.x == 0)                                                                    \
        for (int k_ = 0; k_ < 8; k_++) P.stamps[(1u << 20) + (base) + (uint64_t)blockIdx.x * 8 + k_] = tst_acc[k_];
#else
#define TST_DECL
#define TST(k)
#define TST_FLUSH(base)
#endif
#ifndef PV_WIN
#define PV_WIN 128
#endif
#ifndef PV_WPE
#define PV_WPE 4
#endif
#define PV_WINW (PV_WIN / 4)
#define PV_NWIN 192
#define PV_NOUT 6144

__device__ __forceinline__ uint32_t pv_ld32(const uint8_t *base, uint64_t off)
{
    const uint32_t *p = reinterpret_cast<const uint32_t *>(base + (off & ~3ull));
    uint32_t lo = p[0], hi = p[1];
    return __builtin_amdgcn_alignbyte(hi, lo, (uint32_t)(off & 3));
}
__device__ __forceinline__ uint32_t pv_clz64(uint64_t x) { return (uint32_t)__clzll((long long)x); }
__device__ __forceinline__ uint32_t pv_alignbyte(uint32_t hi, uint32_t lo, uint32_t sh) { return __builtin_amdgcn_alignbyte(hi, lo, sh); }
#define PV_FN __device__ __forceinline__
#define PV_CREF(T) const PV_C T &
#include "pv_parse.h"
#include <type_traits>

namespace {

struct GAcc {
    const uint8_t *R;
    PV_FN uint32_t u32(uint64_t off) const { return pv_ld32(R, off); }
    PV_FN uint32_t u32a(uint64_t off) const { return *reinterpret_cast<const uint32_t *>(R + off); }
    PV_FN uint32_t u8(uint64_t off) const { return R[off]; }
};

struct TAcc {
    const uint8_t *R;
    const uint32_t *L;
    uint64_t gbase;
    uint32_t lim, mul, add;
    PV_FN uint32_t u32(uint64_t off) const
    {
        uint64_t rel = off - gbase;
        if (rel < lim) {
            uint32_t r = (uint32_t)rel;
            uint32_t d = (r >> 2) * mul + add;
            return __builtin_amdgcn_alignbyte(L[d + mul], L[d], r & 3);
        }
        return pv_ld32(R, off);
    }
    PV_FN uint32_t u32a(uint64_t off) const
    {
        uint64_t rel = off - gbase;
        if (rel < lim) return L[(uint32_t)(rel >> 2) * mul + add];
        return *reinterpret_cast<const uint32_t *>(R + off);
    }
    PV_FN uint32_t u8(uint64_t off) const
    {
        uint64_t rel = off - gbase;
        if (rel < lim) {
            uint32_t r = (uint32_t)rel;
            return (L[(r >> 2) * mul + add] >> ((r & 3) * 8)) & 0xff;
        }
        return R[off];
    }
};

struct LAcc {
    const uint32_t *L;
    uint64_t gbase;
    uint32_t mul, add;
    PV_FN uint32_t u32(uint64_t off) const
    {
        const uint32_t r = (uint32_t)(off - gbase), d = (r >> 2) * mul + add;
        return __builtin_amdgcn_alignbyte(L[d + mul], L[d], r & 3);
    }
    PV_FN uint32_t u32a(uint64_t off) const { return L[((uint32_t)(off - gbase) >> 2) * mul + add]; }
    PV_FN uint32_t u8(uint64_t off) const
    {
        const uint32_t r = (uint32_t)(off - gbase);
        return (L[(r >> 2) * mul + add] >> ((r & 3) * 8)) & 0xff;
    }
};

struct LAccT {
    const uint32_t *L;
    uint64_t gbase;
    uint32_t mul, add;
    uint32_t *hi;
    PV_FN uint32_t u32(uint64_t off) const
    {
        const uint32_t r = (uint32_t)(off - gbase), d = (r >> 2) * mul + add;
        *hi = max(*hi, ((r >> 2) + 2) * 4);
        return __builtin_amdgcn_alignbyte(L[d + mul], L[d], r & 3);
    }
    PV_FN uint32_t u32a(uint64_t off) const
    {
        const uint32_t r = (uint32_t)(off - gbase);
        *hi = max(*hi, ((r >> 2) + 1) * 4);
        return L[(r >> 2) * mul + add];
    }
    PV_FN uint32_t u8(uint64_t off) const
    {
        const uint32_t r = (uint32_t)(off - gbase);
        *hi = max(*hi, ((r >> 2) + 1) * 4);
        return (L[(r >> 2) * mul + add] >> ((r & 3) * 8)) & 0xff;
    }
// ... 1548 lines not shown
PV_FN FastRec fast_fields(const RecW &r, const HostNets &h)
{
    FastRec f;
    f.caplen = r.w[2];
    const uint32_t w3 = r.w[7], w4 = r.w[8], w5 = r.w[9];
    const uint32_t proto = w5 >> 24;
    f.ok = (f.caplen >= 34) & ((w3 & 0xffffffu) == 0x450008u) & (proto != 4) & (proto != 41);
    const uint32_t total = ((w4 & 0xff) << 8) | ((w4 >> 8) & 0xff);
    const uint32_t frag = ((w5 & 0xff) << 8) | ((w5 >> 8) & 0xff);
    const uint32_t l = f.caplen - 14;
    const uint32_t len = (total != 0 && total < l) ? total : l;
    const uint32_t pll = len - 20;
    const bool l4ok = (len > 20) & !(frag & 0x3fff);
    const bool udp = l4ok & (proto == 17) & (pll >= 8);
    const bool tcp = l4ok & (proto == 6) & (pll >= 20);
    f.l4 = udp ? 17u : (tcp ? 6u : 0u);
    f.syn = tcp ? (r.w[15] >> 25) & 1 : 0u;
    f.l4len = pll;
    const uint32_t dst = hit4(h, r.at(46)), src = hit4(h, r.at(42));
    f.dir = dst ? 0u : (src ? 1u : 2u);
    return f;
}
PV_FN uint32_t dns_port_bf(uint32_t pw)
{
    const uint32_t sport = ((pw & 0xff) << 8) | ((pw >> 8) & 0xff);
    const uint32_t dport = ((pw >> 8) & 0xff00) | (pw >> 24);
    const bool dd = (dport == 53) | (dport == 5353) | (dport == 5355) | (dport == 53000);
    const bool sd = (sport == 53) | (sport == 5353) | (sport == 5355) | (sport == 53000);
    return dd ? sport : (sd ? dport : 0u);
}
PV_FN Parsed fast_parsed(const FastRec &f, const RecW &r, uint32_t ts_nano, uint64_t off)
{
    Parsed o;
    o.caplen = f.caplen;
    o.sec = r.w[0];
    o.nsec = ts_nano ? (int32_t)r.w[1] : (int32_t)(r.w[1] * 1000u);
    o.frame = off + 16;
    o.l3 = 4; o.l4 = (uint8_t)f.l4; o.has4 = 1; o.has6 = 0; o.syn = (uint8_t)f.syn; o.dir = (uint8_t)f.dir;
    o.v4 = o.frame + 14; o.v6 = 0;
    o.l4off = f.l4 ? o.frame + 34 : 0;
    o.l4len = f.l4 ? f.l4len : 0;
    return o;
}
__device__ __forceinline__ SlowOut net_slow_p(const PvParams *__restrict__ Pp, const SAcc R, uint64_t off, uint64_t i)
{
    PV_CREF(PvParams) P = *(const PV_C PvParams *)Pp;
    NetK K;
    K.recs = P.recs; K.offs = P.offs; K.n = P.n; K.rec_bytes = P.rec_bytes; K.gbase = P.gbase;
    K.sum = P.sum; K.cpc = P.cpc; K.iplog = P.iplog; K.dq = P.dq; K.flags = P.flags;
    K.n_shift = 0; K.skip_before = 0; K.slot0 = P.slot_of[0];
    K.net_groups = P.net_groups; K.dbg = 0; K.net_filter_all = 0;
    K.n_dshift = P.n_dshift; K.dskip_before = P.dskip_before;
    K.tcp_emit = P.tcp_emit; K.tseg_cap = P.tseg_cap; K.tseg = P.tseg; K.tseg_cnt = P.tseg_cnt; K.tmask = P.tmask;
    K.ndeep_net = nullptr; K.ndeep_dns = nullptr; K.gfilt = nullptr;
    return net_slow_body(R, parse_cfg(P), P, K, off, i, K.slot0, true);
}

#ifndef PV_REG_MINW
#define PV_REG_MINW 2
#endif
struct NetRegState {
    uint32_t hist[PV_HBINS];
    uint32_t nd, nx, ns;
    int64_t dord[PV_MAX_SHIFTS];
};
__device__ __forceinline__ void win_load(const PV_G uint8_t *recs, uint32_t off, uint4 (&W)[5])
{
    const PV_G uint4 *p = reinterpret_cast<const PV_G uint4 *>(recs + (off & ~3u));
#pragma unroll
    for (int j = 0; j < 5; j++) W[j] = p[j];
}
__device__ __forceinline__ void win_words(const uint4 (&W)[5], uint32_t sh, RecW &r)
{
    uint32_t x[17];
#pragma unroll
    for (int k = 0; k < 4; k++) { x[4 * k] = W[k].x; x[4 * k + 1] = W[k].y; x[4 * k + 2] = W[k].z; x[4 * k + 3] = W[k].w; }
    x[16] = W[4].x;
#pragma unroll
    for (int j = 0; j < 16; j++) r.w[j] = __builtin_amdgcn_alignbyte(x[j + 1], x[j], sh);
}
#ifdef PV_TSTAMPS
#define PV_TST_NET ((1u << 20) + (1u << 18))
#define TST_WALL(P, k) if (threadIdx.x == 0) (P).stamps[PV_TST_NET + 4ull * blockIdx.x + (k)] = wall_clock64();
#else
#define TST_WALL(P, k)
#endif
__device__ __forceinline__ void net_ranges(PV_CREF(PvParams) P, bool contig, uint32_t &lb0, uint32_t &lb1, uint32_t &step)
{
    lb0 = blockIdx.x; lb1 = P.grid_main; step = gridDim.x;
    if (contig) { lb0 = min(blockIdx.x * P.cb_fan, P.grid_main); lb1 = min(lb0 + P.cb_fan, P.grid_main); step = 1; }
}
template <uint32_t NW, bool TC = false, bool FUSE = false>
__device__ __forceinline__ void net_fast_reg(const PvParams *__restrict__ Pp)
{
    PV_CREF(PvParams) P = *(const PV_C PvParams *)Pp;
    __shared__ NetRegState S;
    TST_WALL(P, 0)
    const uint32_t wave = __builtin_amdgcn_readfirstlane(threadIdx.x >> 6), lane = threadIdx.x & 63;
    for (uint32_t b = threadIdx.x; b < PV_HBINS; b += (FUSE ? 64u * NW : blockDim.x)) S.hist[b] = 0;
    if (threadIdx.x == 0) { S.nd = 0; S.nx = 0; S.ns = 0; }
    if (threadIdx.x < PV_MAX_SHIFTS) S.dord[threadIdx.x] = P.dpos[threadIdx.x];
    __syncthreads();
    const PV_G uint8_t *const recs = P.recs;
    const bool compact = P.ip_compact;
    const PV_G uint32_t *const offs = P.offs;
    const uint64_t n = P.n, last = n - 1;
    const uint32_t slot = P.slot_of[0];
    const uint32_t groups = P.net_groups;
    const bool tops = groups & PV_NET_TOP_IPS_BIT, card = groups & PV_NET_CARDINALITY_BIT;
    const uint32_t ts_nano = P.ts_nano;
    HostNets h;
    {
        const uint32_t n4 = P.nets.n4;
        h.a0 = P.nets.v4_addr[0]; h.m0 = P.nets.v4_mask[0]; h.e0 = n4 > 0 ? ~0u : 0u;
        h.a1 = P.nets.v4_addr[1]; h.m1 = P.nets.v4_mask[1]; h.e1 = n4 > 1 ? ~0u : 0u;
    }
    const uint64_t nwt = (n + PV_WT - 1) / PV_WT;
    uint64_t cd = 0, cl = 0;
    NetCtr c;
    c.zero();
    bool any = false;
#ifdef PV_RANGE_AB
    uint32_t lb0, lb1, lbstep;
    net_ranges(P, FUSE || P.net_contig, lb0, lb1, lbstep);
    for (uint32_t lb = lb0; lb < lb1; lb += lbstep) {
#else
    for (uint32_t lb = FUSE ? blockIdx.x * P.cb_fan : blockIdx.x; lb < (FUSE ? min(blockIdx.x * P.cb_fan + P.cb_fan, P.grid_main) : P.grid_main);
         lb += FUSE ? 1u : gridDim.x) {
#endif
    const uint64_t wbeg = (uint64_t)lb * P.wt_per_block;
    const uint64_t wend = min<uint64_t>(wbeg + P.wt_per_block, nwt);
    const uint32_t ntl = wend > wbeg + wave ? (uint32_t)((wend - wbeg - wave + NW - 1) / NW) : 0u;
    any |= ntl != 0;
    auto tile_of = [&](uint32_t k) -> uint64_t { return wbeg + wave + (uint64_t)NW * min(k, ntl - 1); };
    auto off_of = [&](uint32_t k) -> uint32_t { return offs[min<uint64_t>(tile_of(k) * PV_WT + lane, last)]; };
    PV_G uint64_t *const trash = P.trash + ((uint64_t)blockIdx.x * NW + wave) * 256;
    auto tile = [&](uint32_t k, uint32_t off, const uint4 (&W)[5]) {
        const bool live = k < ntl;
        const uint64_t t = tile_of(k);
        const uint64_t r0 = t * PV_WT, i = r0 + lane;
        const bool active = live && i < n;
        RecW rw;
        win_words(W, off & 3, rw);
        const FastRec f = fast_fields(rw, h);
        const bool fast = active & (f.ok != 0);
        const uint64_t slowm = __ballot(active & !fast);
        cd += fast ? 1ull << (f.dir * 16) : 0ull;
        cl += fast ? (1ull << (f.l4 == 17 ? 0u : (f.l4 == 6 ? 16u : 32u))) + ((uint64_t)f.syn << 48) : 0ull;
        uint32_t hv = fast ? f.caplen : PV_NOH;
        const uint32_t ip = f.dir == 0 ? rw.at(42) : rw.at(46);
        const bool ipok = fast & (f.dir != 2) & (ip != 0);
        uint64_t ek = tops && ipok ? ((uint64_t)slot << 60) | ((uint64_t)TM_IPV4 << 56) | ((uint64_t)card << 33) |
                                         ((uint64_t)f.dir << 32) | ip
                                   : 0ull;
        if (card && !tops) {
            if (ipok) {
                uint64_t h1, h2;
                murmur_8((uint64_t)(int64_t)(int32_t)ip, h1, h2);
                __hip_atomic_fetch_min(P.cpc + (uint64_t)slot * PV_MIN_WORDS + (uint64_t)(f.dir == 0 ? CPC_SRC : CPC_DST) * PV_CPC_COUPONS +
                                           cpc_coupon(h1, h2),
                                       (int64_t)(P.gbase + i), __ATOMIC_RELAXED, __HIP_MEMORY_SCOPE_AGENT);
            }
        }
        const uint32_t port = (fast & (f.l4 == 17)) ? dns_port_bf(rw.at(50)) : 0u;
        DnsMsgW dm{};
        bool isdns = port != 0;
        if (__ballot(isdns)) {
            if (isdns) {
                const Parsed o = fast_parsed(f, rw, ts_nano, off);
                uint32_t dp = 0;
                for (uint32_t q = 0; q < P.n_dshift; q++) dp += (int64_t)(4 * i) >= S.dord[q];
                const SAcc R{recs, nullptr, 0, 0, 0, 1};
                DnsMsg d = dns_msg_of(P, R, o, i, port, dp, dp >= P.dskip_before, false);
                d.fkey = fast_flowkey(rw);
                dm = msg_words(d);
            }
        }
        bool istcp = fast & (f.l4 == 6), hasseg = false;
        PvTcpSeg seg;
        const uint32_t temit = P.tcp_emit;
        if (temit && __ballot(istcp)) {
            if (istcp) hasseg = tcp_seg_fast(rw, fast_parsed(f, rw, ts_nano, off), i, seg);
        }
        if (slowm) {
            uint32_t q = 0;
            if (lane == 0) q = atomicAdd(&S.ns, (uint32_t)__popcll(slowm));
            q = __builtin_amdgcn_readlane(q, 0) + __builtin_amdgcn_mbcnt_hi((uint32_t)(slowm >> 32), __builtin_amdgcn_mbcnt_lo((uint32_t)slowm, 0u));
            if (active && !fast) P.slow_list[wbeg * PV_WT + q] = (uint32_t)i;
        }
        if (__ballot(hv != PV_NOH && hv > 65535)) {
            if (hv != PV_NOH && hv > 65535) { atomicOr(P.flags, PVF_BIG_CAPLEN); hv = 65535; }
        }
        hist_add(S.hist, P.sum + (uint64_t)slot * PV_SUM_WORDS + PV_OFF_PAYLOAD, hv, lane);
        const uint64_t m = __ballot(isdns);
        if (m) {
            uint32_t q = 0;
            if (lane == 0) q = atomicAdd(&S.nd, (uint32_t)__popcll(m));
            q = __builtin_amdgcn_readlane(q, 0);
            const uint32_t below = __builtin_amdgcn_mbcnt_hi((uint32_t)(m >> 32), __builtin_amdgcn_mbcnt_lo((uint32_t)m, 0u));
            if (isdns) {
                PV_G uint4 *dd = reinterpret_cast<PV_G uint4 *>(P.dq) + 2 * (wbeg * PV_WT + q + below);
                dd[0] = dm.a;
                dd[1] = dm.b;
            }
        }
        if (TC || tops) {
            if (TC || compact) {
                const bool v4 = ek && ((ek >> 32) & ~1ull) == (P.ip_base >> 32);
                const uint64_t xm = __ballot(active && ek && !v4);
                const uint64_t dbit = __ballot(v4 && ((ek >> 32) & 1));
                if (TC) {
                    PV_G uint32_t *const l32 = live ? P.iplog32 + i : reinterpret_cast<PV_G uint32_t *>(trash) + lane;
                    PV_G uint64_t *const ldw = live ? P.ipdir + t : trash + 32;
                    *l32 = active && v4 ? (uint32_t)ek : 0u;
                    *ldw = dbit;
                } else if (live) {
                    if (active) P.iplog32[i] = v4 ? (uint32_t)ek : 0u;
                    if (lane == 0) P.ipdir[t] = dbit;
                }
                if (xm) {
                    uint32_t q = 0;
                    if (lane == 0) q = atomicAdd(&S.nx, (uint32_t)__popcll(xm));
                    q = __builtin_amdgcn_readlane(q, 0);
                    const uint32_t below = __builtin_amdgcn_mbcnt_hi((uint32_t)(xm >> 32), __builtin_amdgcn_mbcnt_lo((uint32_t)xm, 0u));
                    if (active && ek && !v4) {
                        P.iplog[wbeg * PV_WT + q + below] = ek;
                        P.ipx_rep[wbeg * PV_WT + q + below] = (uint32_t)i;
                    }
                }
            } else if (active) {
                P.iplog[i] = ek;
            }
        }
        if (temit) {
            const uint64_t tm = __ballot(istcp);
            if (tm) {
                if (lane == 0) P.tmask[t] = tm;
                tcp_seg_store(P.tseg, P.tseg_cnt, P.tseg_cap, hasseg, seg, lane);
            }
        }
    };
    if (ntl) {
        uint4 W0[5], W1[5], W2[5];
        uint32_t o0 = off_of(0), o1 = off_of(1), o2 = off_of(2);
        win_load(recs, o0, W0);
        win_load(recs, o1, W1);
        for (uint32_t k = 0; k < ntl; k += 3) {
            const uint32_t oN = off_of(k + 3);
            win_load(recs, o2, W2);
            tile(k, o0, W0);
            const uint32_t oN1 = off_of(k + 4);
            win_load(recs, oN, W0);
            o0 = oN;
            tile(k + 1, o1, W1);
            const uint32_t oN2 = off_of(k + 5);
            win_load(recs, oN1, W1);
            o1 = oN1;
            tile(k + 2, o2, W2);
            o2 = oN2;
        }
    }
    if constexpr (FUSE) __builtin_amdgcn_s_waitcnt(PV_WAIT_VMCNT0);
    lds_barrier();
    if (threadIdx.x == 0) {
        P.mq_cnt[lb] = 0;
        P.dq_cnt[lb] = S.nd;
        if (compact) P.ipx_cnt[lb] = S.nx;
        P.slow_cnt[lb] = S.ns;
        if (S.nd) atomicAdd(P.n_dns, S.nd);
        if (S.ns) atomicAdd(P.n_slow, S.ns);
        S.nd = 0;
        S.nx = 0;
        S.ns = 0;
    }
    lds_barrier();
    }
    {
        const uint32_t fin = (uint32_t)(cd & 0xffff), fout = (uint32_t)((cd >> 16) & 0xffff), funk = (uint32_t)((cd >> 32) & 0xffff);
        const uint32_t nf = fin + fout + funk;
        c.nev += nf; c.n4 += nf;
        c.nin += fin; c.nout += fout; c.nunk += funk;
        c.nudp += (uint32_t)(cl & 0xffff); c.ntcp += (uint32_t)((cl >> 16) & 0xffff);
        c.noth += (uint32_t)((cl >> 32) & 0xffff); c.nsyn += (uint32_t)(cl >> 48);
    }
    NetK K;
    K.sum = P.sum; K.net_groups = groups; K.net_filter_all = 0; K.gfilt = nullptr;
    if (any) knet_flush(K, slot, c);
    lds_barrier();
    for (uint32_t b = threadIdx.x; b < PV_HBINS; b += (FUSE ? 64u * NW : blockDim.x))
        if (S.hist[b]) ksum_add(K, slot, PV_OFF_PAYLOAD + b, S.hist[b]);
    TST_WALL(P, 1)
}

#ifndef PV_SPAN_MAX
#define PV_SPAN_MAX 6144
#endif
typedef uint32_t v4u32 __attribute__((ext_vector_type(4)));
struct NetSpanState {
    uint32_t hist[PV_HBINS];
    uint32_t nd, ns;
    int64_t dord[PV_MAX_SHIFTS];
    v4u32 buf[4][PV_SPAN_MAX / 16 + 8];
};
struct SpanX {
    v4u32 v0, v1, v2, v3, v4, v5;
};
__device__ __forceinline__ void span_load(const PV_G uint8_t *recs, uint32_t o, uint32_t lane, SpanX &X, uint32_t &b)
{
    const uint32_t o0 = __builtin_amdgcn_readfirstlane(o), o63 = __builtin_amdgcn_readlane(o, 63);
    const uint32_t b16 = o0 & ~15u;
    const uint32_t len = o63 + 80u - b16;
    const PV_G v4u32 *ps = reinterpret_cast<const PV_G v4u32 *>(recs + b16);
    const bool sp = o63 >= o0 && len <= PV_SPAN_MAX && !__ballot(o < o0 || o > o63);
    b = sp ? b16 : 0xffffffffu;
    const uint32_t lim = sp ? len : 0u;
#define PV_SPAN_LD(j) X.v##j = ps[16u * (lane + 64u * j) < lim ? lane + 64u * j : 0u]
    PV_SPAN_LD(0); PV_SPAN_LD(1); PV_SPAN_LD(2); PV_SPAN_LD(3); PV_SPAN_LD(4); PV_SPAN_LD(5);
#undef PV_SPAN_LD
}
extern "C" __global__ void __launch_bounds__(256) __attribute__((amdgpu_waves_per_eu(PV_REG_MINW))) pv_net_kernel_span(const PvParams *__restrict__ Pp)
{
    PV_CREF(PvParams) P = *(const PV_C PvParams *)Pp;
    __shared__ NetSpanState S;
    constexpr uint32_t NW = 4;
    const uint32_t wave = __builtin_amdgcn_readfirstlane(threadIdx.x >> 6), lane = threadIdx.x & 63;
    for (uint32_t b = threadIdx.x; b < PV_HBINS; b += blockDim.x) S.hist[b] = 0;
    if (threadIdx.x == 0) { S.nd = 0; S.ns = 0; }
    if (threadIdx.x < PV_MAX_SHIFTS) S.dord[threadIdx.x] = P.dpos[threadIdx.x];
    __syncthreads();
    const PV_G uint8_t *const recs = P.recs;
    const PV_G uint32_t *const offs = P.offs;
    const uint64_t n = P.n, last = n - 1;
    const uint32_t slot = P.slot_of[0];
    const uint32_t groups = P.net_groups;
    const bool card = groups & PV_NET_CARDINALITY_BIT;
    const uint32_t ts_nano = P.ts_nano;
    HostNets h;
    {
        const uint32_t n4 = P.nets.n4;
        h.a0 = P.nets.v4_addr[0]; h.m0 = P.nets.v4_mask[0]; h.e0 = n4 > 0 ? ~0u : 0u;
        h.a1 = P.nets.v4_addr[1]; h.m1 = P.nets.v4_mask[1]; h.e1 = n4 > 1 ? ~0u : 0u;
    }
    const uint64_t nwt = (n + PV_WT - 1) / PV_WT;
    uint64_t cd = 0, cl = 0;
    v4u32 *Lq = S.buf[wave];
// ... 725 lines not shown
}
template <class St>
__device__ __forceinline__ void comb_chit(St &S, uint32_t pos, uint32_t rel, uint32_t rel0)
{
    const uint32_t sh = 16u * (pos & 1u);
    atomicAdd(&S.ccnt[pos >> 1], 1u << sh);
    if (rel < rel0) {
        uint32_t old = S.crep[pos >> 1];
        while (rel < ((old >> sh) & 0xffffu)) {
            const uint32_t prev = atomicCAS(&S.crep[pos >> 1], old, (old & ~(0xffffu << sh)) | rel << sh);
            if (prev == old) break;
            old = prev;
        }
    }
}
template <class St>
__device__ __forceinline__ bool comb_cbucket(St &S, uint32_t b, uint32_t par, uint32_t ip, uint32_t rel)
{
    const uint4 *kp = reinterpret_cast<const uint4 *>(&S.ckey[b]);
    const uint4 lo = kp[0], hi = kp[1];
    const uint32_t cur4[4] = {par ? lo.y : lo.x, par ? lo.w : lo.z, par ? hi.y : hi.x, par ? hi.w : hi.z};
#pragma unroll
    for (int j = 0; j < 4; j++) {
        const uint32_t s = b + 2u * j + par;
        uint32_t cur = cur4[j];
        if (cur == 0) {
            const uint32_t prev = atomicCAS(&S.ckey[s], 0u, ip);
            cur = prev == 0 ? ip : prev;
        }
        if (cur == ip) {
            comb_chit(S, s, rel, 0xffffffffu);
            return true;
        }
    }
    return false;
}
template <uint32_t CN2, class St>
__device__ __forceinline__ void comb_cadd_pre(PV_CREF(PvParams) P, St &S, PV_G ulonglong2 *sp, uint32_t ip, uint32_t dir,
                                              uint32_t base, uint32_t rel, uint32_t pos, uint32_t cur0, uint32_t rel0)
{
    uint32_t cur = cur0;
    if (cur == 0) {
        const uint32_t prev = atomicCAS(&S.ckey[pos], 0u, ip);
        cur = prev == 0 ? ip : prev;
        rel0 = 0xffffffffu;
    }
    if (cur == ip) {
        comb_chit(S, pos, rel, rel0);
        return;
    }
    for (uint32_t g = 1; g <= 4; g++)
        if (comb_cbucket(S, ((pos & ~7u) + 8u * g) & (CN2 - 1), pos & 1u, ip, rel)) return;
    comb_spill(P, S, sp, P.ip_base | (uint64_t)dir << 32 | ip, 1u, base + rel);
}

__device__ __forceinline__ uint32_t block_excl_scan(uint32_t v, uint32_t *wsum, uint32_t &total)
{
    const uint32_t lane = threadIdx.x & 63, wv = threadIdx.x >> 6, nw = (blockDim.x + 63) >> 6;
    uint32_t incl = v;
#pragma unroll
    for (int o = 1; o < 64; o <<= 1) {
        const uint32_t t = __shfl_up(incl, o, 64);
        if (lane >= (uint32_t)o) incl += t;
    }
    if (lane == 63) wsum[wv] = incl;
    __syncthreads();
    uint32_t base = 0, tot = 0;
    for (uint32_t k = 0; k < nw; k++) {
        const uint32_t s = wsum[k];
        if (k < wv) base += s;
        tot += s;
    }
    __syncthreads();
    total = tot;
    return base + incl - v;
}

template <bool FUSE, class T>
__device__ __forceinline__ T ld_own(const PV_G T *p)
{
    if constexpr (FUSE) return __hip_atomic_load(p, __ATOMIC_RELAXED, __HIP_MEMORY_SCOPE_AGENT);
    else return *p;
}
template <uint32_t CN, class St>
__device__ __forceinline__ void comb_init(St &S, uint32_t nreg, uint32_t tid, uint32_t nt)
{
    for (uint32_t j = tid; j < CN; j += nt) { S.key[j] = 0; S.cnt[j] = 0; S.rep[j] = 0xffffffffu; }
    for (uint32_t r = tid; r < nreg; r += nt) {
        S.h[r] = 0;
        if (!(r & 1)) S.tb[r >> 1] = 0;
    }
    if (tid == 0) S.nsp = 0;
}
template <uint32_t CN, class St>
__device__ __forceinline__ void comb_crange_own(PV_CREF(PvParams) P, St &S, PV_G ulonglong2 *sp, uint32_t gr, uint32_t cbase,
                                                uint32_t tid, uint32_t bd)
{
    const PV_G uint32_t *ip4 = P.iplog32;
    uint64_t a, z;
    wg_records(P, gr, a, z);
    const uint32_t nn = (uint32_t)(z - a), ra = (uint32_t)(a - cbase);
    for (uint32_t j0 = tid; j0 < nn; j0 += PV_CB_U * bd) {
        uint32_t ipv[PV_CB_U];
        uint64_t dw[PV_CB_U];
#pragma unroll
        for (int u = 0; u < PV_CB_U; u++) {
            const uint32_t j = j0 + u * bd;
            ipv[u] = j < nn ? ld_own<true>(ip4 + a + j) : 0u;
            dw[u] = j < nn ? ld_own<true>(P.ipdir + ((a + j) >> 6)) : 0ull;
        }
        uint32_t dir[PV_CB_U], pos[PV_CB_U], cur[PV_CB_U], rp[PV_CB_U];
#pragma unroll
        for (int u = 0; u < PV_CB_U; u++) {
            const uint64_t r = a + j0 + (uint64_t)u * bd;
            dir[u] = (uint32_t)(dw[u] >> (r & 63)) & 1u;
            pos[u] = comb_cpos<2 * CN>(ipv[u], dir[u]);
            cur[u] = ipv[u] ? S.ckey[pos[u]] : 0u;
            rp[u] = ipv[u] ? (S.crep[pos[u] >> 1] >> (16u * (pos[u] & 1u))) & 0xffffu : 0u;
        }
#pragma unroll
        for (int u = 0; u < PV_CB_U; u++)
            if (ipv[u]) comb_cadd_pre<2 * CN>(P, S, sp, ipv[u], dir[u], cbase, ra + j0 + u * bd, pos[u], cur[u], rp[u]);
    }
}
template <uint32_t CN, uint32_t NR, bool FUSE = false>
__device__ __forceinline__ void topn_combine(PV_CREF(PvParams) P, const PvParams *__restrict__ Pp = nullptr)
{
    using St = CombState<CN, NR>;
    __shared__ St S;
    constexpr uint32_t CK = 16;
    constexpr bool CAN = CN * 2 == CK * PV_CB_THREADS && NR <= 2048;
    bool early = false;
    if constexpr (FUSE) {
        static_assert(sizeof(St) + sizeof(NetRegState) <= 160 * 1024, "pv_net_combine_plain: the Net state and the combine table in one CU's LDS");
        constexpr uint32_t NETW = 4;
        const uint32_t e0 = blockIdx.x * P.cb_fan, e1 = min(e0 + P.cb_fan, P.grid_main);
        uint64_t ea = 0, ez = 0, eb, ey = 0;
        if (e1 > e0) { wg_records(P, e0, ea, ez); wg_records(P, e1 - 1, eb, ey); }
#ifndef PV_FUSE_NO_EARLY
        early = CAN && P.cb_compact && e1 > e0 + 1 && P.ip_compact && (P.net_groups & PV_NET_TOP_IPS_BIT) && blockDim.x == PV_CB_THREADS &&
                ey - ea <= 65535;
#endif
        if (__builtin_amdgcn_readfirstlane(threadIdx.x >> 6) < NETW) {
            net_fast_reg<NETW, true, true>(Pp);
            __builtin_amdgcn_s_waitcnt(PV_WAIT_VMCNT0);
        } else {
            const uint32_t tid = threadIdx.x - 64u * NETW, nt = blockDim.x - 64u * NETW;
            lds_barrier();
            comb_init<CN>(S, 2u << P.reg_log2, tid, nt);
            for (uint32_t gr = e0; gr < e1; gr++) {
                lds_barrier();
                lds_barrier();
                if (early && gr + 1 < e1)
                    comb_crange_own<CN>(P, S, reinterpret_cast<PV_G ulonglong2 *>(P.tp_buf) + (uint64_t)e0 * P.mq_cap, gr, (uint32_t)ea, tid, nt);
            }
            lds_barrier();
        }
        __syncthreads();
        TST_WALL(P, 2)
    }
    if constexpr (!FUSE) {
        if (P.plain_chain && (*P.n_dns | *P.n_slow)) return;
    }
    TST_DECL
    const uint32_t nreg = 2u << P.reg_log2;
    const uint32_t g0 = blockIdx.x * P.cb_fan, g1 = min(g0 + P.cb_fan, P.grid_main);
    if constexpr (FUSE) {
        uint32_t bad = 0;
        for (uint32_t gr = g0; gr < g1; gr++) bad |= ld_own<true>(P.dq_cnt + gr) | ld_own<true>(P.slow_cnt + gr);
        if (bad) return;
    }
    const uint64_t wbase = (uint64_t)g0 * P.mq_cap;
    PV_G ulonglong2 *sp = reinterpret_cast<PV_G ulonglong2 *>(P.tp_buf) + wbase;
    PV_G ulonglong2 *out = reinterpret_cast<PV_G ulonglong2 *>(P.cb) + wbase;
    uint32_t cbase = 0;
    uint32_t other = 1;
    if constexpr (CAN) {
        if (P.cb_compact && g1 - g0 > 1 && P.ip_compact && (P.net_groups & PV_NET_TOP_IPS_BIT) && blockDim.x == PV_CB_THREADS) {
            uint64_t a0, z0, a1, z1;
            wg_records(P, g0, a0, z0);
            wg_records(P, g1 - 1, a1, z1);
            other = z1 - a0 > 65535 ? 1u : 0u;
            for (uint32_t gr = g0; gr < g1; gr++) other |= ld_own<FUSE>(P.mq_cnt + gr) | ld_own<FUSE>(P.ipx_cnt + gr);
            cbase = (uint32_t)a0;
        }
    }
    if constexpr (!FUSE) {
    for (uint32_t j = threadIdx.x; j < CN; j += blockDim.x) { S.key[j] = 0; S.cnt[j] = 0; S.rep[j] = 0xffffffffu; }
    for (uint32_t r = threadIdx.x; r < nreg; r += blockDim.x) {
        S.h[r] = 0;
        if (!(r & 1)) S.tb[r >> 1] = 0;
    }
    if (threadIdx.x == 0) S.nsp = 0;
    }
    const bool compact = CAN && __builtin_amdgcn_readfirstlane(other) == 0;
    if constexpr (!FUSE) __syncthreads();
    TST(0)
    if (compact) {
        if constexpr (CAN) {
            const PV_G uint32_t *ip4 = P.iplog32;
            for (uint32_t gr = FUSE && early ? g1 - 1 : g0; gr < g1; gr++) {
                uint64_t a, z;
                wg_records(P, gr, a, z);
                const uint32_t nn = (uint32_t)(z - a), bd = blockDim.x, ra = (uint32_t)(a - cbase);
                for (uint32_t j0 = threadIdx.x; j0 < nn; j0 += PV_CB_U * bd) {
                    uint32_t ipv[PV_CB_U];
                    uint64_t dw[PV_CB_U];
#pragma unroll
                    for (int u = 0; u < PV_CB_U; u++) {
                        const uint32_t j = j0 + u * bd;
                        ipv[u] = j < nn ? ld_own<FUSE>(ip4 + a + j) : 0u;
                        dw[u] = j < nn ? ld_own<FUSE>(P.ipdir + ((a + j) >> 6)) : 0ull;
                    }
                    uint32_t dir[PV_CB_U], pos[PV_CB_U], cur[PV_CB_U], rp[PV_CB_U];
#pragma unroll
                    for (int u = 0; u < PV_CB_U; u++) {
                        const uint64_t r = a + j0 + (uint64_t)u * bd;
                        dir[u] = (uint32_t)(dw[u] >> (r & 63)) & 1u;
                        pos[u] = comb_cpos<2 * CN>(ipv[u], dir[u]);
                        cur[u] = ipv[u] ? S.ckey[pos[u]] : 0u;
                        rp[u] = ipv[u] ? (S.crep[pos[u] >> 1] >> (16u * (pos[u] & 1u))) & 0xffffu : 0u;
                    }
#pragma unroll
                    for (int u = 0; u < PV_CB_U; u++)
                        if (ipv[u]) comb_cadd_pre<2 * CN>(P, S, sp, ipv[u], dir[u], cbase, ra + j0 + u * bd, pos[u], cur[u], rp[u]);
                }
            }
        }
    } else
    for (uint32_t gr = g0; gr < g1; gr++) {
    const uint32_t cnt = ld_own<FUSE>(P.mq_cnt + gr);
    const PV_G uint64_t *q = P.mq + (uint64_t)gr * P.mq_cap * 2;
    batched<8>(cnt, [&](uint64_t j) { return PV_E16(q)[j]; },
               [&](uint64_t, ulonglong2 e) { comb_add<CN>(P, S, sp, e.x, (uint32_t)e.y, (uint32_t)(e.y >> 32)); });
    if (P.net_groups & PV_NET_TOP_IPS_BIT) {
        uint64_t a, z;
        wg_records(P, gr, a, z);
        const PV_G uint64_t *ipl = P.iplog + a;
        if (P.ip_compact) {
            const PV_G uint32_t *ip4 = P.iplog32;
            const uint64_t nn = z - a, bd = blockDim.x;
            const uint64_t ipb = P.ip_base;
            for (uint64_t j0 = threadIdx.x; j0 < nn; j0 += (uint64_t)PV_CB_U * bd) {
                uint32_t ipv[PV_CB_U];
                uint64_t dw[PV_CB_U];
#pragma unroll
                for (int u = 0; u < PV_CB_U; u++) {
                    const uint64_t j = j0 + (uint64_t)u * bd;
                    ipv[u] = j < nn ? ld_own<FUSE>(ip4 + a + j) : 0u;
                    dw[u] = j < nn ? ld_own<FUSE>(P.ipdir + ((a + j) >> 6)) : 0ull;
                }
                uint64_t ck[PV_CB_U], cur[PV_CB_U];
                uint32_t pos[PV_CB_U], rp[PV_CB_U];
#pragma unroll
                for (int u = 0; u < PV_CB_U; u++) {
                    const uint64_t r = a + j0 + (uint64_t)u * bd;
                    ck[u] = ipb | ((dw[u] >> (r & 63)) & 1) << 32 | ipv[u];
                    pos[u] = (uint32_t)(fmix64(ck[u]) >> 20) & (CN - 1);
                    cur[u] = ipv[u] ? S.key[pos[u]] : 0ull;
                    rp[u] = ipv[u] ? S.rep[pos[u]] : 0u;
                }
#pragma unroll
                for (int u = 0; u < PV_CB_U; u++)
                    if (ipv[u]) comb_add_pre<CN>(P, S, sp, ck[u], 1u, (uint32_t)(a + j0 + (uint64_t)u * bd), pos[u], cur[u], rp[u]);
            }
            const uint32_t nx = ld_own<FUSE>(P.ipx_cnt + gr);
            for (uint32_t q = threadIdx.x; q < nx; q += blockDim.x)
                comb_add<CN>(P, S, sp, ld_own<FUSE>(ipl + q), 1u, ld_own<FUSE>(P.ipx_rep + a + q));
        } else {
            batched<PV_CB_U>(z - a, [&](uint64_t j) { return ipl[j]; }, [&](uint64_t j, uint64_t e) {
                if (e) comb_add<CN>(P, S, sp, e, 1u, (uint32_t)(a + j));
            });
        }
    }
    }
    if (threadIdx.x == 0) S.hm = 0;
    __syncthreads();
    TST(1)
    uint32_t rk[CK / 2] = {};
    if (compact) {
        if constexpr (CAN) {
            const uint64_t tk = P.ip_base & (0xffull << 56);
#pragma unroll
            for (uint32_t k = 0; k < CK; k++) {
                const uint32_t ip = S.ckey[threadIdx.x + k * PV_CB_THREADS];
                const uint32_t r = ip ? comb_count(P, S, tk | ip) : 0u;
                rk[k / 2] = k & 1 ? rk[k / 2] | r << 16 : r;
            }
        }
    } else
    for (uint32_t j = threadIdx.x; j < CN; j += blockDim.x)
        if (S.key[j]) comb_count(P, S, comb_entry(S.key[j], S.cnt[j], S.rep[j]).x);
    __syncthreads();
    TST(2)
    const uint32_t per = (nreg + blockDim.x - 1) / blockDim.x;
    const uint32_t r0 = min(threadIdx.x * per, nreg), r1 = min(r0 + per, nreg);
    uint32_t s = 0;
    for (uint32_t r = r0; r < r1; r++) s += S.h[r];
    {
        const uint32_t hb = s ? 1u << (r0 >> P.reg_log2) : 0u;
        const uint64_t b0 = __ballot(hb & 1), b1 = __ballot(hb & 2);
        if ((threadIdx.x & 63) == 0 && (b0 | b1)) atomicOr(&S.hm, (b0 ? 1u : 0u) | (b1 ? 2u : 0u));
    }
    uint32_t total;
    uint32_t run = block_excl_scan(s, S.wsum, total);
    const uint32_t hm = S.hm;
    if (threadIdx.x < 2 && ((hm >> threadIdx.x) & 1)) atomicOr(P.tp_hands, 1u << threadIdx.x);
    if (threadIdx.x == 0) P.cb_hm[blockIdx.x] = hm;
    const uint32_t ng8 = (P.cb_grid + 7) / 8;
    PV_G uint64_t *col = P.cb_run + (blockIdx.x % 8) * ng8 + blockIdx.x / 8;
    for (uint32_t r = r0; r < r1; r++) {
        const uint32_t c = S.h[r];
        if ((hm >> (r >> P.reg_log2)) & 1) col[(uint64_t)r * 8 * ng8] = pv_run_word(run, c, (S.tb[r >> 1] >> (16u * (r & 1u))) & 0xffffu);
        S.h[r] = run;
        run += c;
    }
    lds_barrier();
    TST(3)
    if (compact) {
        if constexpr (CAN) {
#pragma unroll 1
            for (uint32_t q = 0; q < PV_CB_OSWEEP; q++)
#pragma unroll
            for (uint32_t k = 0; k < CK; k++) {
                const uint32_t j = threadIdx.x + k * PV_CB_THREADS, sh = 16u * (j & 1u);
                const uint32_t ip = S.ckey[j];
                if (!ip) continue;
                if (PV_CB_OSWEEP > 1 && ((((rk[k / 2] >> (16u * (k & 1u))) & 0xffffu) * PV_CB_OSWEEP) >> P.reg_log2) != q) continue;
                const uint64_t ck = P.ip_base | (uint64_t)((j ^ (uint32_t)__popc(ip)) & 1u) << 32 | ip;
                const ulonglong2 e = comb_entry(ck, (S.ccnt[j >> 1] >> sh) & 0xffffu, cbase + ((S.crep[j >> 1] >> sh) & 0xffffu));
                out[atomicAdd(&S.h[(rk[k / 2] >> (16u * (k & 1u))) & 0xffffu], 1u)] = e;
            }
        }
    } else
    for (uint32_t j = threadIdx.x; j < CN; j += blockDim.x)
        if (S.key[j]) {
            const ulonglong2 e = comb_entry(S.key[j], S.cnt[j], S.rep[j]);
            out[atomicAdd(&S.h[run_key(P, e.x)], 1u)] = e;
        }
    const uint32_t nsp = S.nsp;
    batched<8>(nsp, [&](uint64_t j) { return sp[j]; },
               [&](uint64_t, ulonglong2 e) { out[atomicAdd(&S.h[run_key(P, e.x)], 1u)] = e; });
    if (threadIdx.x == 0) P.cb_cnt[blockIdx.x] = total;
#ifdef PV_TSTAMPS
    __syncthreads();
#endif
    TST(4)
    TST_FLUSH(0)
    if constexpr (FUSE) { TST_WALL(P, 3) }
}
#ifndef PV_CB_CN
#define PV_CB_CN 8192
#endif
static_assert(PV_SLOTS == 16, "pv_topn_combine folds a table bit to 16 bits a region");
extern "C" __global__ void __launch_bounds__(PV_CB_THREADS) pv_topn_combine(const PvParams *__restrict__ Pp)
{
    PV_CREF(PvParams) P = *(const PV_C PvParams *)Pp;
    topn_combine<PV_CB_CN, 2048>(P);
}
extern "C" __global__ void __launch_bounds__(PV_CB_THREADS) pv_net_combine_plain(const PvParams *__restrict__ Pp)
{
    PV_CREF(PvParams) P = *(const PV_C PvParams *)Pp;
    topn_combine<PV_CB_CN, 2048, true>(P, Pp);
}
extern "C" __global__ void __launch_bounds__(PV_CB_THREADS) pv_topn_combine_r12(const PvParams *__restrict__ Pp)
{
    PV_CREF(PvParams) P = *(const PV_C PvParams *)Pp;
    topn_combine<2048, 2u << PV_MAX_REGIONS_LOG2>(P);
}

#define PV_MG_THREADS 512
#ifndef PV_MG_U2
#define PV_MG_U2 4
#endif
#ifndef PV_MG_SEEN
#define PV_MG_SEEN 1
#endif
#define PV_MG_NN 640
#define PV_CREATED (1ull << 63)
#define PV_MV4 (1ull << 62)
#define PV_MN1 (0xffffffull << 32)
#define PV_DL0 (0xffffffffull << 32)
__device__ __forceinline__ bool mv4_key(uint64_t k) { return PV_KEY_METRIC(k) == TM_IPV4 && !((k >> 40) & 1); }
__device__ __forceinline__ uint64_t mv4_norm(uint64_t w) { return w & ~(PV_CREATED | ((w & PV_MV4) ? PV_MN1 : 0ull)); }
struct MergeState {
    alignas(16) uint64_t key[PV_RS];
    uint64_t dl[PV_RS];
    uint32_t nrep[PV_MG_NN];
    uint16_t nidx[PV_MG_NN];
    uint32_t nnew, nbase, ncr;
    uint32_t ip4c;
};
struct MergeRuns {
    uint32_t start[PV_MAX_GRID + 8];
    uint32_t pref[PV_MAX_GRID + 9];
    uint16_t list[PV_MAX_GRID + 8];
    uint32_t wsum[16];
    uint32_t tabs;
};
static_assert(2 * PV_MG_THREADS >= (PV_MAX_GRID + 7) / 8 * 8, "two runs per merge thread");
static_assert(sizeof(MergeState) + sizeof(MergeRuns) <= 80 * 1024, "pv_topn_merge: two workgroups per CU");
extern "C" uint32_t pv_topn_merge_threads() { return PV_MG_THREADS; }
extern "C" __global__ void __launch_bounds__(PV_MG_THREADS) __attribute__((amdgpu_waves_per_eu(4))) pv_topn_merge(const PvParams *__restrict__ Pp)
{
    PV_CREF(PvParams) P = *(const PV_C PvParams *)Pp;
    const uint32_t rk = blockIdx.x;
    const uint32_t r = rk & ((1u << P.reg_log2) - 1);
    const uint32_t hd = rk >> P.reg_log2;
    if (P.plain_chain && (*P.n_dns | *P.n_slow)) return;
    if (!((*P.tp_hands >> hd) & 1)) return;
    if (P.xmerge && (r < P.x_lo || r >= P.x_hi)) return;
    __shared__ MergeRuns U;
    __shared__ MergeState S;
    TST_DECL
    const uint32_t ng8 = (P.cb_grid + 7) / 8, ng = 8 * ng8;
    const uint64_t lcap = (uint64_t)P.cb_fan * P.mq_cap;
    const uint32_t rsl = P.tcap_log2 - P.reg_log2;
    const uint32_t rs = 1u << rsl;
    const uint32_t tbg = hd ? PV_SLOTS + P.dslot_of[0] : P.slot_of[0];
    const uint64_t rbg = ((uint64_t)tbg << P.tcap_log2) + ((uint64_t)r << rsl);
    const bool pf = rs == PV_RS;
    if (pf) {
        static_assert(PV_RS * 8 == 32 * 1024 && PV_MG_THREADS == 512, "four pieces per wave");
        const uint32_t wv = threadIdx.x >> 6, ln = threadIdx.x & 63;
#pragma unroll
        for (int q = 0; q < 4; q++) {
            const uint32_t pc = wv * 4 + q;
            dma16(P.tkeys + rbg + pc * 128 + ln * 2, lds_addr(&S.key[pc * 128]));
        }
    }
    uint32_t n;
    {
        uint32_t c0 = 0, c1 = 0, tb = 0;
        if (threadIdx.x == 0) U.tabs = 0;
        const uint32_t i0 = 2 * threadIdx.x;
        if (i0 < ng) {
            const ulonglong2 v = *reinterpret_cast<const PV_G ulonglong2 *>(P.cb_run + (uint64_t)rk * ng + i0);
            const uint32_t w0 = (i0 % ng8) * 8 + i0 / ng8, w1 = ((i0 + 1) % ng8) * 8 + (i0 + 1) / ng8;
            const bool h0 = w0 < P.cb_grid && ((P.cb_hm[w0] >> hd) & 1);
            const bool h1 = w1 < P.cb_grid && ((P.cb_hm[w1] >> hd) & 1);
            U.start[i0] = (uint32_t)v.x & 0xffffffu;
            U.start[i0 + 1] = (uint32_t)v.y & 0xffffffu;
            U.list[i0] = (uint16_t)w0;
            U.list[i0 + 1] = (uint16_t)w1;
            c0 = h0 ? (uint32_t)(v.x >> 24) & 0xffffffu : 0u;
            c1 = h1 ? (uint32_t)(v.y >> 24) & 0xffffffu : 0u;
// ... 1719 lines not shown
```

Before: 29070 Mpkt/s.

## Pass IP log through an LDS ring between net and combine waves in fused kernel

Adds a fused net+combine kernel variant in which the net-parsing waves write each tile's IPv4 keys and direction bits into a double-buffered shared-memory ring. The combine waves consume them section by section, so the per-record iplog32/ipdir global writes and their later re-reads are dropped. The ring is only selected after two consecutive plain batches and when the compact range fits in 16 bits. If a later slow path needs the IP log, a separate pv_net_iplog kernel re-derives it from the records. Each section adds barriers coupling producer and consumer waves, which can stall the pipelined load loop.

```diff
diff --git a/include/pvgpu.h b/include/pvgpu.h
--- a/include/pvgpu.h
+++ b/include/pvgpu.h
@@ -257,6 +257,7 @@
 int pv_kernel_timing(pv_ctx *ctx, double *total_ms, uint64_t *launches, int reset);
 int pv_chain_stats(pv_ctx *ctx, uint64_t out[4], int reset);
 int pv_fuse_stats(pv_ctx *ctx, uint64_t out[2], int reset);
+int pv_ring_stats(pv_ctx *ctx, uint64_t out[2], int reset);
 
 typedef struct pv_geodb pv_geodb;
 enum pv_geodb_kind { PV_GEODB_CITY = 0, PV_GEODB_ASN = 1 };
diff --git a/pktvisor_amd/__init__.py b/pktvisor_amd/__init__.py
--- a/pktvisor_amd/__init__.py
+++ b/pktvisor_amd/__init__.py
@@ -167,7 +167,8 @@
            "pv_topn_x_candidates", "pv_topn_x_names", "pv_topn_x_view", "pv_values_x_select", "pv_comm_values_select",
            "pv_slow_x_finish", "pv_comm_slow_finish", "pv_geodb_open", "pv_geodb_open_file", "pv_geodb_close",
            "pv_geodb_last_error", "pv_geodb_entries", "pv_geodb_hash", "pv_geodb_hashes", "pv_set_net_filters", "pv_geodb_entry", "pv_geodb_lookup", "pv_set_geodb",
-           "pv_geodb_lookup_device", "pv_set_dhcp", "pv_dhcp_timing", "pv_set_bgp", "pv_bgp_timing", "pv_chain_stats", "pv_fuse_stats"]
+           "pv_geodb_lookup_device", "pv_set_dhcp", "pv_dhcp_timing", "pv_set_bgp", "pv_bgp_timing", "pv_chain_stats", "pv_fuse_stats",
+           "pv_ring_stats"]
 PV_GEODB_CITY, PV_GEODB_ASN = 0, 1
 ALLREDUCE_FN = ctypes.CFUNCTYPE(ctypes.c_int, ctypes.POINTER(ctypes.c_uint64), ctypes.c_size_t, ctypes.c_int, ctypes.c_void_p)
 PV_HANDLER_NET, PV_HANDLER_DNS, PV_HANDLER_DHCP, PV_HANDLER_BGP = 1, 2, 4, 8
@@ -358,6 +359,8 @@
         lib.pv_chain_stats.argtypes = [P, ctypes.POINTER(U64), ctypes.c_int]
     if hasattr(lib, "pv_fuse_stats"):
         lib.pv_fuse_stats.argtypes = [P, ctypes.POINTER(U64), ctypes.c_int]
+    if hasattr(lib, "pv_ring_stats"):
+        lib.pv_ring_stats.argtypes = [P, ctypes.POINTER(U64), ctypes.c_int]
     _lib = lib
     return lib
 
@@ -778,6 +781,11 @@
         self._check(self.lib.pv_fuse_stats(self.ctx, out, int(reset)), "pv_fuse_stats")
         return tuple(int(v) for v in out)
 
+    def ring_stats(self, reset: bool = False):
+        out = (ctypes.c_uint64 * 2)()
+        self._check(self.lib.pv_ring_stats(self.ctx, out, int(reset)), "pv_ring_stats")
+        return tuple(int(v) for v in out)
+
     def set_net_filters(self, geoloc_notfound=False, asn_notfound=False, only_geoloc_prefix=None, only_asn_number=None):
         f = pv_net_filters(int(bool(geoloc_notfound)), int(bool(asn_notfound)))
         keep = []
diff --git a/pktvisor_amd/csrc/pv_host.cpp b/pktvisor_amd/csrc/pv_host.cpp
--- a/pktvisor_amd/csrc/pv_host.cpp
+++ b/pktvisor_amd/csrc/pv_host.cpp
@@ -2150,6 +2150,11 @@
     const bool timed = n && c->timing_every && (c->timing_ctr++ % c->timing_every) == 0;
     hipEvent_t e0 = timed ? c->ev_start : nullptr, e1 = timed ? c->ev_stop : nullptr;
     if (timed) fuse = false;
+    bool ring = fuse && P.cb_compact && c->cb_plain_run >= 2 && (uint64_t)P.cb_fan * P.wt_per_block * 64 <= 65535;
+    if (ring) {
+        const char *fr = getenv("PV_FUSE_RING");
+        if (fr && atoi(fr) == 0) ring = false;
+    }
     if (P.gfilt && n) {
         PvGeoArgs G{};
         for (int k = 0; k < 2; k++) {
@@ -2169,7 +2174,8 @@
     else if (general) hipExtLaunchKernelGGL(pv_net_kernel, dim3(grid), dim3(PV_NET_THREADS), 0, st, e0, e1, 0, dp);
     else if (lean) {
         hipEvent_t l1 = plain ? e1 : (hipEvent_t) nullptr;
-        if (fuse) hipLaunchKernelGGL(pv_net_combine_plain, dim3(P.cb_grid), dim3(PV_CB_THREADS), 0, st, dp);
+        if (ring) hipLaunchKernelGGL(pv_net_combine_ring, dim3(P.cb_grid), dim3(PV_CB_THREADS), 0, st, dp);
+        else if (fuse) hipLaunchKernelGGL(pv_net_combine_plain, dim3(P.cb_grid), dim3(PV_CB_THREADS), 0, st, dp);
         else if (span) hipExtLaunchKernelGGL(pv_net_kernel_span, dim3(reg_grid), dim3(PV_NET_THREADS), 0, st, e0, l1, 0, dp);
         else if (tc) hipExtLaunchKernelGGL(pv_net_kernel_reg_tc, dim3(reg_grid), dim3(PV_NET_THREADS), 0, st, e0, l1, 0, dp);
         else hipExtLaunchKernelGGL(pv_net_kernel_reg, dim3(reg_grid), dim3(PV_NET_THREADS), 0, st, e0, l1, 0, dp);
@@ -2242,6 +2248,7 @@
         topn_stage(fuse);
         c->chain_n[0]++;
         if (fuse) c->fuse_n[0]++;
+        if (ring) c->nolog_n[0]++;
     }
 
     HP(14);
@@ -2252,6 +2259,10 @@
         P.plain_chain = 0;
         c->h_params->plain_chain = 0;
         if (!hip_ok(e = upload_params(c->d_params, c->h_params, sizeof P, st))) return c->hipfail(e, "parameter upload");
+        if (ring) {
+            c->nolog_n[1]++;
+            hipLaunchKernelGGL(pv_net_iplog, dim3(c->cus * 4), dim3(256), 0, st, dp);
+        }
         hipLaunchKernelGGL(pv_net_slow_list, dim3(c->cus * 2), dim3(256), 0, st, dp);
         dns_stage();
         topn_stage();
@@ -2265,6 +2276,7 @@
     if (n) {
         c->dns_heavy = (uint64_t)status[ST_NDNS] * 2 > n;
         c->cb_plain = lean && status[ST_NDNS] == 0 && status[ST_NSLOW] == 0;
+        c->cb_plain_run = c->cb_plain ? std::min(c->cb_plain_run + 1, 2u) : 0;
     }
     if (status[ST_FLAGS] & PVF_NAMES_PENDING) {
         for (uint32_t t = 0; t < PV_TABLES; t++)
@@ -2326,7 +2338,12 @@
         hipDeviceGetAttribute(&khz, hipDeviceAttributeWallClockRate, c->device);
         if (lean && hip_ok(hipMemcpy(nv.data(), c->d_stamps + (1u << 20) + (1u << 18), nv.size() * 8, hipMemcpyDeviceToHost)) && nv[0]) {
             uint64_t first = ~0ull;
-            for (uint32_t w = 0; w < reg_grid; w++) first = std::min(first, nv[w * 4]);
+            std::vector<uint32_t> xcc(reg_grid);
+            for (uint32_t w = 0; w < reg_grid; w++) {
+                xcc[w] = (uint32_t)(nv[w * 4] >> 60);
+                nv[w * 4] &= ~(0xfull << 60);
+                first = std::min(first, nv[w * 4]);
+            }
             const double us = khz > 0 ? 1000.0 / khz : 0.01;
             fprintf(stderr, "pv_tstamps net (%u wg, %s):", reg_grid, fuse ? "fused" : "pair");
             static const char *nm[4] = {"start", "net_end", "handover", "end"};
@@ -2337,6 +2354,16 @@
                 if (v.empty()) continue;
                 std::sort(v.begin(), v.end());
                 fprintf(stderr, " %s min=%.2f med=%.2f max=%.2f us", nm[k], v.front(), v[v.size() / 2], v.back());
+            }
+            fprintf(stderr, "\n");
+            fprintf(stderr, "pv_tstamps net_end by xcc:");
+            for (uint32_t x = 0; x < 16; x++) {
+                std::vector<double> v;
+                for (uint32_t w = 0; w < reg_grid; w++)
+                    if (xcc[w] == x && nv[w * 4 + 1]) v.push_back((double)(nv[w * 4 + 1] - first) * us);
+                if (v.empty()) continue;
+                std::sort(v.begin(), v.end());
+                fprintf(stderr, " x%u(n=%zu) %.0f/%.0f/%.0f", x, v.size(), v.front(), v[v.size() / 2], v.back());
             }
             fprintf(stderr, "\n");
             hipMemset(c->d_stamps + (1u << 20) + (1u << 18), 0, nv.size() * 8);
@@ -2653,6 +2680,16 @@
     for (int k = 0; k < 2; k++) {
         if (out) out[k] = c->fuse_n[k];
         if (reset) c->fuse_n[k] = 0;
+    }
+    return 0;
+}
+
+extern "C" int pv_ring_stats(pv_ctx *c, uint64_t out[2], int reset)
+{
+    std::lock_guard<std::mutex> g(c->mu);
+    for (int k = 0; k < 2; k++) {
+        if (out) out[k] = c->nolog_n[k];
+        if (reset) c->nolog_n[k] = 0;
     }
     return 0;
 }
diff --git a/pktvisor_amd/csrc/pv_host.h b/pktvisor_amd/csrc/pv_host.h
--- a/pktvisor_amd/csrc/pv_host.h
+++ b/pktvisor_amd/csrc/pv_host.h
@@ -140,6 +140,8 @@
 extern "C" __global__ void pv_dns_prescan(const PvParams *P);
 extern "C" __global__ void pv_topn_combine(const PvParams *P);
 extern "C" __global__ void pv_net_combine_plain(const PvParams *P);
+extern "C" __global__ void pv_net_combine_ring(const PvParams *P);
+extern "C" __global__ void pv_net_iplog(const PvParams *P);
 extern "C" __global__ void pv_topn_combine_r12(const PvParams *P);
 extern "C" __global__ void pv_topn_merge(const PvParams *P);
 extern "C" __global__ void pv_topn_names_sfx(const PvParams *P);
@@ -622,6 +624,8 @@
     bool cb_plain = false;
     uint64_t chain_n[4] = {0, 0, 0, 0};
     uint64_t fuse_n[2] = {0, 0};
+    uint32_t cb_plain_run = 0;
+    uint64_t nolog_n[2] = {0, 0};
     int dns_wg_per_cu = 1;
     const char *net_kernel = "none";
     uint64_t *d_dq = nullptr;
diff --git a/pktvisor_amd/csrc/pv_kernels.hip b/pktvisor_amd/csrc/pv_kernels.hip
--- a/pktvisor_amd/csrc/pv_kernels.hip
+++ b/pktvisor_amd/csrc/pv_kernels.hip
@@ -63,6 +63,7 @@
 #define PV_FN __device__ __forceinline__
 #define PV_CREF(T) const PV_C T &
 #include "pv_parse.h"
+#include "pv_ring.h"
 #include <type_traits>
 
 namespace {
@@ -1777,7 +1778,10 @@
 #ifdef PV_TSTAMPS
 #define PV_TST_NET ((1u << 20) + (1u << 18))
 #define TST_WALL(P, k) if (threadIdx.x == 0) (P).stamps[PV_TST_NET + 4ull * blockIdx.x + (k)] = wall_clock64();
+#define TST_WALL_XCC(P) \
+    if (threadIdx.x == 0) (P).stamps[PV_TST_NET + 4ull * blockIdx.x] = (wall_clock64() & ~(0xfull << 60)) | (uint64_t)__builtin_amdgcn_s_getreg(20 | (3 << 11)) << 60;
 #else
+#define TST_WALL_XCC(P)
 #define TST_WALL(P, k)
 #endif
 __device__ __forceinline__ void net_ranges(PV_CREF(PvParams) P, bool contig, uint32_t &lb0, uint32_t &lb1, uint32_t &step)
@@ -1785,12 +1789,19 @@
     lb0 = blockIdx.x; lb1 = P.grid_main; step = gridDim.x;
     if (contig) { lb0 = min(blockIdx.x * P.cb_fan, P.grid_main); lb1 = min(lb0 + P.cb_fan, P.grid_main); step = 1; }
 }
-template <uint32_t NW, bool TC = false, bool FUSE = false>
-__device__ __forceinline__ void net_fast_reg(const PvParams *__restrict__ Pp)
-{
+struct FuseRing {
+    struct Sec {
+        uint32_t ip[PV_RING_SLOTS][PV_WT];
+        uint64_t dm[PV_RING_SLOTS];
+    } sec[2];
+};
+template <uint32_t NW, bool TC = false, bool FUSE = false, bool RING = false>
+__device__ __forceinline__ void net_fast_reg(const PvParams *__restrict__ Pp, FuseRing *ring = nullptr)
+{
+    static_assert(!RING || (FUSE && TC && NW == PV_RING_WAVES), "the ring is the fused kernel's");
     PV_CREF(PvParams) P = *(const PV_C PvParams *)Pp;
     __shared__ NetRegState S;
-    TST_WALL(P, 0)
+    TST_WALL_XCC(P)
     const uint32_t wave = __builtin_amdgcn_readfirstlane(threadIdx.x >> 6), lane = threadIdx.x & 63;
     for (uint32_t b = threadIdx.x; b < PV_HBINS; b += (FUSE ? 64u * NW : blockDim.x)) S.hist[b] = 0;
     if (threadIdx.x == 0) { S.nd = 0; S.nx = 0; S.ns = 0; }
@@ -1815,6 +1826,7 @@
     NetCtr c;
     c.zero();
     bool any = false;
+    uint32_t secn = 0;
 #ifdef PV_RANGE_AB
     uint32_t lb0, lb1, lbstep;
     net_ranges(P, FUSE || P.net_contig, lb0, lb1, lbstep);
@@ -1827,7 +1839,8 @@
     const uint64_t wend = min<uint64_t>(wbeg + P.wt_per_block, nwt);
     const uint32_t ntl = wend > wbeg + wave ? (uint32_t)((wend - wbeg - wave + NW - 1) / NW) : 0u;
     any |= ntl != 0;
-    auto tile_of = [&](uint32_t k) -> uint64_t { return wbeg + wave + (uint64_t)NW * min(k, ntl - 1); };
+    const uint32_t nsk = RING ? pv_ring_sections(wend > wbeg ? (uint32_t)(wend - wbeg) : 0u) * PV_RING_K : 0u;
+    auto tile_of = [&](uint32_t k) -> uint64_t { return wbeg + wave + (uint64_t)NW * min(k, RING && !ntl ? 0u : ntl - 1); };
     auto off_of = [&](uint32_t k) -> uint32_t { return offs[min<uint64_t>(tile_of(k) * PV_WT + lane, last)]; };
     PV_G uint64_t *const trash = P.trash + ((uint64_t)blockIdx.x * NW + wave) * 256;
     auto tile = [&](uint32_t k, uint32_t off, const uint4 (&W)[5]) {
@@ -1904,11 +1917,21 @@
                 const bool v4 = ek && ((ek >> 32) & ~1ull) == (P.ip_base >> 32);
                 const uint64_t xm = __ballot(active && ek && !v4);
                 const uint64_t dbit = __ballot(v4 && ((ek >> 32) & 1));
-                if (TC) {
+                if constexpr (RING) {
+                    FuseRing::Sec &rs = ring->sec[secn & 1];
+                    const uint32_t q = pv_ring_slot(wave, k);
+                    rs.ip[q][lane] = active && v4 ? (uint32_t)ek : 0u;
+                    if (lane == 0) rs.dm[q] = dbit;
+                } else if (TC) {
+#ifdef PV_FUSE_NOSTORE
+                    if constexpr (!FUSE)
+#endif
+                    {
                     PV_G uint32_t *const l32 = live ? P.iplog32 + i : reinterpret_cast<PV_G uint32_t *>(trash) + lane;
                     PV_G uint64_t *const ldw = live ? P.ipdir + t : trash + 32;
                     *l32 = active && v4 ? (uint32_t)ek : 0u;
                     *ldw = dbit;
+                    }
                 } else if (live) {
                     if (active) P.iplog32[i] = v4 ? (uint32_t)ek : 0u;
                     if (lane == 0) P.ipdir[t] = dbit;
@@ -1935,12 +1958,13 @@
             }
         }
     };
-    if (ntl) {
+    static_assert(PV_RING_K == 3, "a section is one turn of the pipeline loop");
+    if (RING ? nsk : ntl) {
         uint4 W0[5], W1[5], W2[5];
         uint32_t o0 = off_of(0), o1 = off_of(1), o2 = off_of(2);
         win_load(recs, o0, W0);
         win_load(recs, o1, W1);
-        for (uint32_t k = 0; k < ntl; k += 3) {
+        for (uint32_t k = 0; k < (RING ? nsk : ntl); k += 3) {
             const uint32_t oN = off_of(k + 3);
             win_load(recs, o2, W2);
             tile(k, o0, W0);
@@ -1953,9 +1977,13 @@
             o1 = oN1;
             tile(k + 2, o2, W2);
             o2 = oN2;
-        }
-    }
-    if constexpr (FUSE) __builtin_amdgcn_s_waitcnt(PV_WAIT_VMCNT0);
+            if constexpr (RING) {
+                lds_barrier();
+                secn++;
+            }
+        }
+    }
+    if constexpr (FUSE && !RING) __builtin_amdgcn_s_waitcnt(PV_WAIT_VMCNT0);
     lds_barrier();
     if (threadIdx.x == 0) {
         P.mq_cnt[lb] = 0;
@@ -2847,6 +2875,15 @@
     if constexpr (FUSE) return __hip_atomic_load(p, __ATOMIC_RELAXED, __HIP_MEMORY_SCOPE_AGENT);
     else return *p;
 }
+template <bool RING>
+__device__ __forceinline__ FuseRing *fuse_ring()
+{
+    if constexpr (RING) {
+        __shared__ FuseRing r;
+        return &r;
+    } else
+        return nullptr;
+}
 template <uint32_t CN, class St>
 __device__ __forceinline__ void comb_init(St &S, uint32_t nreg, uint32_t tid, uint32_t nt)
 {
@@ -2888,7 +2925,7 @@
             if (ipv[u]) comb_cadd_pre<2 * CN>(P, S, sp, ipv[u], dir[u], cbase, ra + j0 + u * bd, pos[u], cur[u], rp[u]);
     }
 }
-template <uint32_t CN, uint32_t NR, bool FUSE = false>
+template <uint32_t CN, uint32_t NR, bool FUSE = false, bool RING = false>
 __device__ __forceinline__ void topn_combine(PV_CREF(PvParams) P, const PvParams *__restrict__ Pp = nullptr)
 {
     using St = CombState<CN, NR>;
@@ -2906,9 +2943,41 @@
         early = CAN && P.cb_compact && e1 > e0 + 1 && P.ip_compact && (P.net_groups & PV_NET_TOP_IPS_BIT) && blockDim.x == PV_CB_THREADS &&
                 ey - ea <= 65535;
 #endif
+        FuseRing *const ring = fuse_ring<RING>();
+        if constexpr (RING) {
+            static_assert(CAN && sizeof(St) + sizeof(NetRegState) + sizeof(FuseRing) <= 160 * 1024, "pv_net_combine_ring: the ring beside them");
+            static_assert(PV_CB_THREADS == 64 * (NETW + PV_RING_SLOTS), "an inserting thread a slot's lane");
+            early = true;
+        }
         if (__builtin_amdgcn_readfirstlane(threadIdx.x >> 6) < NETW) {
-            net_fast_reg<NETW, true, true>(Pp);
+            net_fast_reg<NETW, true, true, RING>(Pp, ring);
             __builtin_amdgcn_s_waitcnt(PV_WAIT_VMCNT0);
+        } else if constexpr (RING) {
+            const uint32_t tid = threadIdx.x - 64u * NETW, nt = blockDim.x - 64u * NETW;
+            const uint32_t slot = tid >> 6, lane = tid & 63;
+            PV_G ulonglong2 *const sp = reinterpret_cast<PV_G ulonglong2 *>(P.tp_buf) + (uint64_t)e0 * P.mq_cap;
+            const uint64_t nwt = (P.n + PV_WT - 1) / PV_WT;
+            lds_barrier();
+            comb_init<CN>(S, 2u << P.reg_log2, tid, nt);
+            uint32_t secn = 0;
+            for (uint32_t gr = e0; gr < e1; gr++) {
+                const uint64_t wbeg = (uint64_t)gr * P.wt_per_block, wend = min<uint64_t>(wbeg + P.wt_per_block, nwt);
+                const uint32_t ns = pv_ring_sections(wend > wbeg ? (uint32_t)(wend - wbeg) : 0u);
+                const uint32_t ra = (uint32_t)(wbeg * PV_WT - ea);
+                for (uint32_t s = 0; s < ns; s++, secn++) {
+                    lds_barrier();
+                    const FuseRing::Sec &rs = ring->sec[secn & 1];
+                    const uint32_t ip = rs.ip[slot][lane];
+                    if (ip) {
+                        const uint32_t dir = (uint32_t)(rs.dm[slot] >> lane) & 1u, pos = comb_cpos<2 * CN>(ip, dir);
+                        comb_cadd_pre<2 * CN>(P, S, sp, ip, dir, (uint32_t)ea, ra + (pv_ring_tile(s, slot) * PV_WT + lane), pos, S.ckey[pos],
+                                              (S.crep[pos >> 1] >> (16u * (pos & 1u))) & 0xffffu);
+                    }
+                }
+                lds_barrier();
+                lds_barrier();
+            }
+            lds_barrier();
         } else {
             const uint32_t tid = threadIdx.x - 64u * NETW, nt = blockDim.x - 64u * NETW;
             lds_barrier();
@@ -2941,7 +3010,7 @@
     uint32_t cbase = 0;
     uint32_t other = 1;
     if constexpr (CAN) {
-        if (P.cb_compact && g1 - g0 > 1 && P.ip_compact && (P.net_groups & PV_NET_TOP_IPS_BIT) && blockDim.x == PV_CB_THREADS) {
+        if (P.cb_compact && (RING || g1 - g0 > 1) && P.ip_compact && (P.net_groups & PV_NET_TOP_IPS_BIT) && blockDim.x == PV_CB_THREADS) {
             uint64_t a0, z0, a1, z1;
             wg_records(P, g0, a0, z0);
             wg_records(P, g1 - 1, a1, z1);
@@ -2958,13 +3027,13 @@
     }
     if (threadIdx.x == 0) S.nsp = 0;
     }
-    const bool compact = CAN && __builtin_amdgcn_readfirstlane(other) == 0;
+    const bool compact = RING || (CAN && __builtin_amdgcn_readfirstlane(other) == 0);
     if constexpr (!FUSE) __syncthreads();
     TST(0)
     if (compact) {
         if constexpr (CAN) {
             const PV_G uint32_t *ip4 = P.iplog32;
-            for (uint32_t gr = FUSE && early ? g1 - 1 : g0; gr < g1; gr++) {
+            for (uint32_t gr = RING ? g1 : (FUSE && early ? g1 - 1 : g0); gr < g1; gr++) {
                 uint64_t a, z;
                 wg_records(P, gr, a, z);
                 const uint32_t nn = (uint32_t)(z - a), bd = blockDim.x, ra = (uint32_t)(a - cbase);
@@ -3127,6 +3196,37 @@
 {
     PV_CREF(PvParams) P = *(const PV_C PvParams *)Pp;
     topn_combine<PV_CB_CN, 2048, true>(P, Pp);
+}
+extern "C" __global__ void __launch_bounds__(PV_CB_THREADS) pv_net_combine_ring(const PvParams *__restrict__ Pp)
+{
+    PV_CREF(PvParams) P = *(const PV_C PvParams *)Pp;
+    topn_combine<PV_CB_CN, 2048, true, true>(P, Pp);
+}
+extern "C" __global__ void __launch_bounds__(256) pv_net_iplog(const PvParams *__restrict__ Pp)
+{
+    PV_CREF(PvParams) P = *(const PV_C PvParams *)Pp;
+    const uint32_t wave = __builtin_amdgcn_readfirstlane(threadIdx.x >> 6), lane = threadIdx.x & 63;
+    const uint64_t n = P.n, nwt = (n + PV_WT - 1) / PV_WT;
+    HostNets h;
+    {
+        const uint32_t n4 = P.nets.n4;
+        h.a0 = P.nets.v4_addr[0]; h.m0 = P.nets.v4_mask[0]; h.e0 = n4 > 0 ? ~0u : 0u;
+        h.a1 = P.nets.v4_addr[1]; h.m1 = P.nets.v4_mask[1]; h.e1 = n4 > 1 ? ~0u : 0u;
+    }
+    for (uint64_t t = (uint64_t)blockIdx.x * 4 + wave; t < nwt; t += (uint64_t)gridDim.x * 4) {
+        const uint64_t i = t * PV_WT + lane;
+        const uint32_t off = P.offs[min<uint64_t>(i, n - 1)];
+        uint4 W[5];
+        win_load(P.recs, off, W);
+        RecW rw;
+        win_words(W, off & 3, rw);
+        const FastRec f = fast_fields(rw, h);
+        const uint32_t ip = f.dir == 0 ? rw.at(42) : rw.at(46);
+        const bool ipok = i < n && f.ok != 0 && f.dir != 2 && ip != 0;
+        const uint64_t dbit = __ballot(ipok && f.dir == 1);
+        P.iplog32[i] = ipok ? ip : 0u;
+        if (lane == 0) P.ipdir[t] = dbit;
+    }
 }
 extern "C" __global__ void __launch_bounds__(PV_CB_THREADS) pv_topn_combine_r12(const PvParams *__restrict__ Pp)
 {
diff --git a/pktvisor_amd/csrc/pv_ring.h b/pktvisor_amd/csrc/pv_ring.h
--- /dev/null
+++ b/pktvisor_amd/csrc/pv_ring.h
@@ -0,0 +1,17 @@
+#pragma once
+#include <stdint.h>
+
+#define PV_RING_WAVES 4
+#define PV_RING_K 3
+#define PV_RING_SLOTS (PV_RING_WAVES * PV_RING_K)
+
+PV_FN uint32_t pv_ring_sections(uint32_t tiles)
+{
+    return (tiles + PV_RING_SLOTS - 1) / PV_RING_SLOTS;
+}
+PV_FN uint32_t pv_ring_section(uint32_t k) { return k / PV_RING_K; }
+PV_FN uint32_t pv_ring_slot(uint32_t w, uint32_t k) { return w * PV_RING_K + k % PV_RING_K; }
+PV_FN uint32_t pv_ring_tile(uint32_t sec, uint32_t slot)
+{
+    return slot / PV_RING_K + PV_RING_WAVES * (sec * PV_RING_K + slot % PV_RING_K);
+}
```

Measured after the change: 30760 Mpkt/s (median of 6 runs). 5.8% higher.
